# chao1224/GeoSSL

Measured on AMD Instinct MI355X. Metric: molecules/s/GPU SchNet+DDM fwd+bwd (QM9-sized, bs=1024); % HBM roofline, higher is better.
Workload: dtype f32

## Files before the change

geossl_amd/NCSN.py:

```python
import ctypes as C
import os

import numpy as np
import torch
from .switches import env as _env
import torch.nn as nn
import torch.nn.functional as F

from . import _lib
from ._lib import call, ptr, stream
from .layout import get_super_edge_layout


class MultiLayerPerceptron(nn.Module):

    def __init__(self, input_dim, hidden_dims, activation="relu", dropout=0):
        super().__init__()
        self.dims = [input_dim] + hidden_dims
        self.activation = getattr(F, activation) if isinstance(activation, str) else None
        self.dropout = nn.Dropout(dropout) if dropout else None
        self.layers = nn.ModuleList()
        for i in range(len(self.dims) - 1):
            self.layers.append(nn.Linear(self.dims[i], self.dims[i + 1]))
        self.reset_parameters()

    def reset_parameters(self):
        for layer in self.layers:
            nn.init.xavier_uniform_(layer.weight)
            nn.init.constant_(layer.bias, 0.0)

    def forward(self, input):
        from .higher_order import _linear_wide
        _lib.require_cuda(input)
        lead = input.shape[:-1]
        x = input.reshape(-1, input.shape[-1])
        for i, layer in enumerate(self.layers):
            x = _linear_wide(x, layer.weight, layer.bias)
            if i < len(self.layers) - 1:
                if self.activation:
                    x = self.activation(x)
                if self.dropout:
                    x = self.dropout(x)
        return x.reshape(*lead, x.shape[-1])


def _head_params(m):
    i, o = m.input_distance_mlp.layers, m.output_mlp.layers
    return [i[0].weight, i[0].bias, i[1].weight, i[1].bias, o[0].weight, o[0].bias, o[1].weight, o[1].bias,
            o[2].weight, o[2].bias]


_FIELDS = ("in_w1", "in_b1", "in_w2", "in_b2", "o1_w", "o1_b", "o2_w", "o2_b", "o3_w", "o3_b")

_SIDE = {"stream": None, "pending": []}


def set_side_stream(stream):
    _SIDE["stream"] = stream


def join_side_stream():
    if _SIDE["pending"]:
        for ev, _keep in _SIDE["pending"]:
            torch.cuda.current_stream().wait_event(ev)
        _SIDE["pending"].clear()


class _NcsnLoss(torch.autograd.Function):
    @staticmethod
    def forward(ctx, h, distance, noise_level, distance_noise, sel, sigmas, anneal_power, out_scale, *params):
        dev = h.device
        S, Fd = sel.S, h.size(1)
        training = ctx.needs_input_grad[0] or any(ctx.needs_input_grad[8:])
        ps = [p.detach().contiguous() for p in params]
        w = _lib.NcsnWeights()
        for name, p in zip(_FIELDS, ps):
            setattr(w, name, ptr(p))
        w.sigmas = ptr(sigmas)
        ctx.grad_slot = getattr(h, "_geossl_grad_slot", None)
        h = h.detach().contiguous()
        loss_e = torch.empty(S, dtype=torch.float32, device=dev)
        sv = None
        saved = {}
        if training:
            saved = dict(a1=torch.empty(S, Fd, dtype=torch.float32, device=dev),
                         a2=torch.empty(S, Fd // 2, dtype=torch.float32, device=dev),
                         pd=torch.empty(S, dtype=torch.float32, device=dev),
                         emb=torch.empty(S, dtype=torch.float32, device=dev),
                         gscale=torch.empty(S, dtype=torch.float32, device=dev))
            sv = _lib.NcsnSaved(*[ptr(saved[k]) for k in ("a1", "a2", "pd", "emb", "gscale")])
        lib = _lib.load()
        nws = max(int(lib.geossl_ddm_loss_fwd_workspace_floats(Fd)), 256)
        ws = (torch.empty if S > 0 else torch.zeros)(nws, dtype=torch.float32, device=dev)
        st = stream()
        call("geossl_ddm_loss_fwd", ptr(h), ptr(sel.batch), ptr(sel.sei0), ptr(sel.sei1), S,
             ptr(distance.contiguous()), ptr(noise_level.contiguous()), ptr(distance_noise.contiguous()), C.byref(w),
             Fd, float(anneal_power), ptr(loss_e), C.byref(sv) if sv is not None else None, ptr(ws), st)
        loss = torch.empty((), dtype=torch.float32, device=dev)
        call("geossl_loss_reduce_partials", ptr(ws), ptr(sel.stats), float(out_scale), ptr(loss), 0, st)
        if training:
            ctx.sel, ctx.ps, ctx.w, ctx.saved, ctx.h = sel, ps, w, saved, h
            ctx.params = params
            ctx.sigmas = sigmas
            ctx.out_scale = float(out_scale)
        return loss

    @staticmethod
    def backward(ctx, gout):
        sel, ps, w, saved, h = ctx.sel, ctx.ps, ctx.w, ctx.saved, ctx.h
        dev = h.device
        S, Fd, N = sel.S, h.size(1), h.size(0)
        st = stream()
        sv = _lib.NcsnSaved(*[ptr(saved[k]) for k in ("a1", "a2", "pd", "emb", "gscale")])
        dfeat = torch.empty(S, Fd, dtype=torch.float32, device=dev)
        demb = torch.empty(S, dtype=torch.float32, device=dev)
        grow = torch.empty(S, dtype=torch.float32, device=dev)
        gout = gout.contiguous().to(torch.float32)
        direct = _lib.direct_grads_enabled(ctx.params)
        grads = [p.grad for p in ctx.params] if direct else [torch.empty_like(p) for p in ps]
        g = _lib.NcsnGrads(*[ptr(t) for t in grads])
        lib = _lib.load()
        acc = 1 if direct else 0
        split = (_env("GEOSSL_NCSN_SPLIT_BWD") is not None or _env("GEOSSL_ARITH_24BIT") is not None
                 or max(S, N) * Fd * 4 >= 2 ** 32)
        if not split:
            ws1 = torch.empty(int(lib.geossl_ddm_loss_bwd_fused_workspace_floats(S, Fd)), dtype=torch.float32, device=dev)
            call("geossl_ddm_loss_bwd_fused", ptr(h), ptr(sel.sei0), ptr(sel.sei1), S, N, Fd, C.byref(w), C.byref(sv),
                 ptr(sel.stats), ctx.out_scale, ptr(gout), ptr(dfeat), ptr(demb), ptr(grow), C.byref(g), ptr(ws1), acc, st)
            dz1 = None
        else:
            dz1 = torch.empty(S, Fd, dtype=torch.float32, device=dev)
            call("geossl_ddm_loss_bwd_rows", C.byref(w), C.byref(sv), S, Fd, ptr(sel.stats), ctx.out_scale, ptr(gout),
                 ptr(dz1), ptr(dfeat), ptr(demb), ptr(grow), st)
        dh = None
        if ctx.needs_input_grad[0]:
            slot = ctx.grad_slot
            dh = slot.rows(N, Fd, torch.float32, dev) if slot is not None else None
            if dh is None:
                dh = torch.empty(N, Fd, dtype=torch.float32, device=dev)
            call("geossl_incidence_gather", ptr(dfeat), ptr(sel.inc_ptr), ptr(sel.inc_idx), N, Fd, ptr(dh), 0, st)
        if split:
            nfl = lib.geossl_ddm_loss_bwd_workspace_floats(S, Fd)
            side = _SIDE["stream"] if direct else None
            if side is None:
                ws = torch.empty(nfl, dtype=torch.float32, device=dev)
                call("geossl_ddm_loss_bwd_weights", ptr(h), ptr(sel.sei0), ptr(sel.sei1), S, Fd, C.byref(w), C.byref(sv),
                     ptr(dz1), ptr(demb), ptr(grow), C.byref(g), ptr(ws), acc, st)
            else:
                main = torch.cuda.current_stream()
                fork = torch.cuda.Event()
                fork.record(main)
                side.wait_event(fork)
                with torch.cuda.stream(side):
                    ws = torch.empty(nfl, dtype=torch.float32, device=dev)
                    call("geossl_ddm_loss_bwd_weights", ptr(h), ptr(sel.sei0), ptr(sel.sei1), S, Fd, C.byref(w),
                         C.byref(sv), ptr(dz1), ptr(demb), ptr(grow), C.byref(g), ptr(ws), 1, stream())
                    done = torch.cuda.Event()
                    done.record(side)
                _SIDE["pending"].append((done, (h, saved, dz1, demb, grow, ws, w, sv, ps, grads)))
        if direct:
            return (dh, None, None, None, None, None, None, None) + (None,) * len(grads)
        return (dh, None, None, None, None, None, None, None) + tuple(grads)


class _NcsnLossPair(torch.autograd.Function):

    @staticmethod
    def forward(ctx, h1, h2, d1, d2, nl1, dn1, nl2, dn2, sel, sigmas, powers, out_scale, npar, *params):
        dev = h1.device
        S, Fd, N = sel.S, h1.size(1), h1.size(0)
        training = ctx.needs_input_grad[0] or ctx.needs_input_grad[1] or any(ctx.needs_input_grad[13:])
        ps = [p.detach().contiguous() for p in params]
        pss = (ps[:npar], ps[npar:])
        dyn = getattr(sel, "dyn", None)
        ctx.dyn = dyn
        if dyn is not None:
            hs = (h1.detach().contiguous(),) * 2
            ctx.grad_slots = (None, None)
        else:
            hs = (h1.detach().contiguous(), h2.detach().contiguous())
            ctx.grad_slots = (getattr(h1, "_geossl_grad_slot", None), getattr(h2, "_geossl_grad_slot", None))
        heads = (_lib.NcsnHeadFwd * 2)()
        keep, saved, ws = [], [], []
        for k, (h, d, nl, dn) in enumerate(((hs[0], d1, nl1, dn1), (hs[1], d2, nl2, dn2))):
            hd = heads[k]
            d, nl, dn = d.contiguous(), nl.contiguous(), dn.contiguous()
            keep += [d, nl, dn]
            for name, p in zip(_FIELDS, pss[k]):
                setattr(hd.w, name, ptr(p))
            hd.w.sigmas = ptr(sigmas[k])
            hd.h, hd.distance, hd.noise_level, hd.distance_noise = ptr(h), ptr(d), ptr(nl), ptr(dn)
            hd.anneal_power = float(powers[k])
            loss_e = torch.empty(S, dtype=torch.float32, device=dev)
            sv = {}
            if training:
                sv = dict(a1=torch.empty(S, Fd, dtype=torch.float32, device=dev),
                          a2=torch.empty(S, Fd // 2, dtype=torch.float32, device=dev),
                          pd=torch.empty(S, dtype=torch.float32, device=dev),
                          emb=torch.empty(S, dtype=torch.float32, device=dev),
                          gscale=torch.empty(S, dtype=torch.float32, device=dev))
                for name in ("a1", "a2", "pd", "emb", "gscale"):
                    setattr(hd.saved, name, ptr(sv[name]))
            w_ = torch.empty(256, dtype=torch.float32, device=dev)
            hd.loss_e, hd.workspace = ptr(loss_e), ptr(w_)
            keep.append(loss_e)
            saved.append(sv)
            ws.append(w_)
        st = stream()
        call("geossl_ddm_loss_fwd2_dyn", C.byref(heads), ptr(sel.batch), ptr(sel.sei0), ptr(sel.sei1), S, Fd,
             None if dyn is None else dyn.n_super, None if dyn is None else dyn.n_atoms, st)
        loss = torch.empty((), dtype=torch.float32, device=dev)
        call("geossl_loss_reduce_partials2", ptr(ws[0]), ptr(ws[1]), ptr(sel.stats), float(out_scale), float(out_scale),
             ptr(loss), st)
        if training:
            ctx.sel, ctx.pss, ctx.saved, ctx.hs, ctx.sigmas = sel, pss, saved, hs, sigmas
            ctx.params, ctx.npar, ctx.out_scale = params, npar, float(out_scale)
        return loss

    @staticmethod
    def backward(ctx, gout):
        sel, pss, saved, hs = ctx.sel, ctx.pss, ctx.saved, ctx.hs
        dev = hs[0].device
        S, Fd, N = sel.S, hs[0].size(1), hs[0].size(0)
        st = stream()
        gout = gout.contiguous().to(torch.float32)
        direct = _lib.direct_grads_enabled(ctx.params)
        grads = [p.grad for p in ctx.params] if direct else [torch.empty_like(p) for p in pss[0] + pss[1]]
        gs = (grads[:ctx.npar], grads[ctx.npar:])
        lib = _lib.load()
        heads = (_lib.NcsnHeadBwd * 2)()
        keep, dhs = [], []
        nws = int(lib.geossl_ddm_loss_bwd_fused_workspace_floats(S, Fd))
        dyn = ctx.dyn
        dh_all = torch.empty(N, Fd, dtype=torch.float32, device=dev) if dyn is not None else None
        for k in range(2):
            hd = heads[k]
            for name, p in zip(_FIELDS, pss[k]):
                setattr(hd.w, name, ptr(p))
            hd.w.sigmas = ptr(ctx.sigmas[k])
            for name in ("a1", "a2", "pd", "emb", "gscale"):
                setattr(hd.saved, name, ptr(saved[k][name]))
            for name, t_ in zip(_FIELDS, gs[k]):
                setattr(hd.grads, name, ptr(t_))
            dfeat = torch.empty(S, Fd, dtype=torch.float32, device=dev)
            demb = torch.empty(S, dtype=torch.float32, device=dev)
            grow = torch.empty(S, dtype=torch.float32, device=dev)
            ws1 = torch.empty(nws, dtype=torch.float32, device=dev)
            slot = ctx.grad_slots[k]
            dh = dh_all if dyn is not None else (slot.rows(N, Fd, torch.float32, dev) if slot is not None else None)
            if dh is None:
                dh = torch.empty(N, Fd, dtype=torch.float32, device=dev)
            hd.h, hd.out_scale, hd.dfeat, hd.demb, hd.grow, hd.workspace, hd.dh = (
                ptr(hs[k]), ctx.out_scale, ptr(dfeat), ptr(demb), ptr(grow), ptr(ws1), ptr(dh))
            keep += [dfeat, demb, grow, ws1]
            dhs.append(dh)
        call("geossl_ddm_loss_bwd_fused2_dyn", C.byref(heads), ptr(sel.sei0), ptr(sel.sei1), S, sel.N if dyn is not None else N,
             Fd, ptr(sel.stats), ptr(gout), ptr(sel.inc_ptr), ptr(sel.inc_idx), 1 if direct else 0,
             None if dyn is None else dyn.n_super, None if dyn is None else dyn.n_atoms, st)
        head = ((dh_all, None) if dyn is not None else (dhs[0], dhs[1])) + (None,) * 11
        if direct:
            return head + (None,) * len(grads)
        return head + tuple(grads)


def ddm_heads_loss(n1, n2, data, h1, distance_1, h2, distance_2, noise_level_1=None, distance_noise_1=None,
                   noise_level_2=None, distance_noise_2=None, out_scale=0.5):
    ok = (isinstance(n1, NCSN_version_03) and isinstance(n2, NCSN_version_03) and n1.emb_dim == n2.emb_dim
          and n1.emb_dim in (32, 64, 128) and not _env("GEOSSL_NCSN_SPLIT_BWD")
          and not _env("GEOSSL_ARITH_24BIT")
          and not _env("GEOSSL_NCSN_SEPARATE_HEADS")
          and (h2 is None or h1.shape == h2.shape) and not distance_1.requires_grad and not distance_2.requires_grad
          and n1 is not n2 and not ({id(p) for p in _head_params(n1)} & {id(p) for p in _head_params(n2)}))
    if ok:
        S_, N_, Fd = data.super_edge_index.size(1), h1.size(0), h1.size(1)
        ok = S_ > 0 and max(S_, N_) * Fd * 4 < 2 ** 32
    bucket = getattr(data, "_bucket", None)
    if bucket is not None and (not ok or h2 is not None):
        raise _lib.GeosslHipError("a capacity-bucket batch needs the paired NCSN heads on one fused feature tensor")
    if not ok:
        return (n1(data, h1, distance_1, noise_level=noise_level_1, distance_noise=distance_noise_1, out_scale=out_scale) +
                n2(data, h2, distance_2, noise_level=noise_level_2, distance_noise=distance_noise_2, out_scale=out_scale))
    _lib.require_cuda(h1, h2, distance_1, distance_2, n1.sigmas, n2.sigmas)
    n1.device = n2.device = n1.sigmas.device
    num_graphs = data.num_graphs
    sel = bucket.sel if bucket is not None else get_super_edge_layout(data.batch, data.super_edge_index, num_graphs)
    draws = []
    for n_, nl, dn, d in ((n1, noise_level_1, distance_noise_1, distance_1), (n2, noise_level_2, distance_noise_2, distance_2)):
        if nl is None:
            nl = torch.randint(0, n_.sigmas.size(0), (num_graphs,), device=n_.sigmas.device)
        if dn is None:
            dn = torch.randn_like(d)
        draws.append((nl, dn))
    p1, p2 = _head_params(n1), _head_params(n2)
    return _NcsnLossPair.apply(h1, h2, distance_1.view(-1), distance_2.view(-1), draws[0][0], draws[0][1].view(-1),
                               draws[1][0], draws[1][1].view(-1), sel, (n1.sigmas.detach(), n2.sigmas.detach()),
                               (n1.anneal_power, n2.anneal_power), out_scale, len(p1), *p1, *p2)


class NCSN_version_03(torch.nn.Module):
    def __init__(self, emb_dim, sigma_begin, sigma_end, num_noise_level, noise_type, anneal_power):
        super().__init__()
        self.anneal_power = anneal_power
        self.noise_type = noise_type
        self.input_distance_mlp = MultiLayerPerceptron(1, [emb_dim, 1], activation="relu")
        self.output_mlp = MultiLayerPerceptron(1 + emb_dim, [emb_dim, emb_dim // 2, 1])
        sigmas = torch.tensor(np.exp(np.linspace(np.log(sigma_begin), np.log(sigma_end), num_noise_level)),
                              dtype=torch.float32)
        self.sigmas = nn.Parameter(sigmas, requires_grad=False)
        self.emb_dim = emb_dim

    def forward(self, data, node_feature, distance, debug=False, noise_level=None, distance_noise=None,
                out_scale=1.0):
        self.device = self.sigmas.device
        _lib.require_cuda(node_feature, distance, self.sigmas)
        if self.emb_dim not in (32, 64, 128):
            raise NotImplementedError("HIP path supports emb_dim in (32, 64, 128)")
        if distance.requires_grad:
            raise NotImplementedError("gradient w.r.t. distance/positions is not built (SURVEY.md §8(f) N3)")
        num_graphs = data.num_graphs
        sel = get_super_edge_layout(data.batch, data.super_edge_index, num_graphs)
        if noise_level is None:
            noise_level = torch.randint(0, self.sigmas.size(0), (num_graphs,), device=self.device)
        if distance_noise is None:
            distance_noise = torch.randn_like(distance)
        if sel.S == 0:
            raise ValueError("batch has no super edges (scatter_add over an empty index fails in the reference too)")
        loss = _NcsnLoss.apply(node_feature, distance.view(-1), noise_level, distance_noise.view(-1), sel,
                               self.sigmas.detach(), self.anneal_power, out_scale, *_head_params(self))
        if debug:
            print("loss", float(loss))
        return loss
```

geossl_amd/_lib.py:

```python
import ctypes as C
import os

import torch

HERE = os.path.dirname(os.path.abspath(__file__))
LIB_PATH = os.path.join(HERE, "lib", "libgeossl_hip.so")

MAX_L = 12
TN_MAX = 32
EPI_BIAS, EPI_SSP, EPI_RESIDUAL, EPI_MUL_DSSP, CHAIN_SAME_INPUT, CHAIN_NEW_INPUT, CHAIN_ADD_PREV = 1, 2, 4, 8, 16, 32, 64
EPI_SILU, EPI_MUL_DSILU = 128, 256

vp = C.c_void_p
i64 = C.c_int64
i32 = C.c_int
f32 = C.c_float
f64 = C.c_double
u64 = C.c_uint64


class FilterWeights(C.Structure):
    _fields_ = [("w1", vp * MAX_L), ("b1", vp * MAX_L), ("w2", vp * MAX_L), ("b2", vp * MAX_L)]


PREPARE_MAX = 64


class PrepareBatch(C.Structure):
    _fields_ = [("W", vp * PREPARE_MAX), ("image", vp * PREPARE_MAX), ("ldw", i32 * PREPARE_MAX), ("tb", i32 * PREPARE_MAX)]


CHAIN_MAX = 5


class ChainStage(C.Structure):
    _fields_ = [("image", vp), ("bias", vp), ("res", vp), ("tprev", vp), ("out", vp), ("ld", i32), ("flags", i32),
                ("xin", vp), ("ldxin", i32), ("pad_", i32), ("out_act", vp)]


class Chain(C.Structure):
    _fields_ = [("nstage", i32), ("st", ChainStage * CHAIN_MAX)]


LOOP_MAX_OPS = 14


class LoopOp(C.Structure):
    _fields_ = [("kind", i32), ("swap", i32), ("X", vp), ("Wf", vp), ("out", vp), ("chain", Chain)]


class FilterGradIn(C.Structure):
    _fields_ = [("x", vp * MAX_L), ("dagg", vp * MAX_L)]


class FilterGradOut(C.Structure):
    _fields_ = [("dw1", vp * MAX_L), ("db1", vp * MAX_L), ("dw2", vp * MAX_L), ("db2", vp * MAX_L)]


class TnBatch(C.Structure):
    _fields_ = [("A", vp * TN_MAX), ("B", vp * TN_MAX), ("dW", vp * TN_MAX), ("db", vp * TN_MAX)]


class NcsnWeights(C.Structure):
    _fields_ = [(k, vp) for k in ("in_w1", "in_b1", "in_w2", "in_b2", "o1_w", "o1_b", "o2_w", "o2_b", "o3_w", "o3_b",
                                  "sigmas")]


class NcsnGrads(C.Structure):
    _fields_ = [(k, vp) for k in ("in_w1", "in_b1", "in_w2", "in_b2", "o1_w", "o1_b", "o2_w", "o2_b", "o3_w", "o3_b")]


class NcsnSaved(C.Structure):
    _fields_ = [(k, vp) for k in ("a1", "a2", "pd", "emb", "gscale")]


class NcsnHeadFwd(C.Structure):
    _fields_ = [("h", vp), ("distance", vp), ("noise_level", vp), ("distance_noise", vp), ("w", NcsnWeights),
                ("saved", NcsnSaved), ("anneal_power", f32), ("pad_", f32), ("loss_e", vp), ("workspace", vp)]


class NcsnHeadBwd(C.Structure):
    _fields_ = [("h", vp), ("w", NcsnWeights), ("saved", NcsnSaved), ("out_scale", f32), ("pad_", f32), ("dfeat", vp),
                ("demb", vp), ("grow", vp), ("grads", NcsnGrads), ("workspace", vp), ("dh", vp)]


COPY_MAX = 8


class CopyBatch(C.Structure):
    _fields_ = [("dst", vp * COPY_MAX), ("src", vp * COPY_MAX), ("bytes", i64 * COPY_MAX)]


class Gather(C.Structure):
    _fields_ = [(k, vp) for k in ("x_src", "pos_src", "src_off", "mol_ptr", "x_dst", "pos_dst", "batch_dst", "se_ptr", "sei0",
                                  "sei1", "pair_ptr2", "pair_i", "pair_j", "inc_ptr", "inc_idx", "e0_src", "e1_src",
                                  "e_src_off", "e_ptr", "e0_dst", "e1_dst", "zero")] + \
               [("zero_count", i64), ("x_cols", i32), ("option", i32)]


class Mask(C.Structure):
    _fields_ = [(k, vp) for k in ("bond_ptr", "bond_dst", "src_n", "mol_id", "keep_in", "keep_out", "e_src_cnt",
                                  "e_count")] + [("seed", u64), ("max_n", i32), ("pad_", i32)]


P = C.POINTER
PROTOTYPES = {
    "geossl_abi_version": (i32, []),
    "geossl_layout_build": (i32, [vp, i64, i64, vp, vp, vp, vp]),
    "geossl_pair_index_fill": (i32, [vp, vp, i64, vp, vp, vp]),
    "geossl_radius_graph_count": (i32, [vp, vp, i64, i32, f32, i32, vp, vp]),
    "geossl_radius_graph_fill": (i32, [vp, vp, i64, i32, f32, i32, vp, vp, vp, vp, vp]),
    "geossl_pair_geometry": (i32, [vp, vp, vp, i64, i32, f32, i32, f32, vp, vp, vp, vp]),
    "geossl_rbf_fwd": (i32, [vp, i64, vp, i32, f32, vp, vp]),
    "geossl_ssp_fwd": (i32, [vp, i64, vp, vp]),
    "geossl_ssp_bwd": (i32, [vp, vp, i64, vp, vp]),
    "geossl_cfconv_filter_fwd": (i32, [vp, vp, i64, P(FilterWeights), i32, i32, i32, vp, f32, vp, vp, vp]),
    "geossl_cfconv_filter_bwd_workspace_floats": (i64, [i64, i32, i32, i32]),
    "geossl_cfconv_filter_bwd": (i32, [vp, vp, vp, vp, vp, i64, i64, P(FilterWeights), P(FilterGradIn), i32, i32, i32, vp,
                                       f32, vp, P(FilterGradOut), vp, i32, vp]),
    "geossl_cfconv_filter_dpos": (i32, [vp, vp, vp, vp, vp, i64, P(FilterWeights), P(FilterGradIn), i32, i32, i32, vp, f32,
                                        f32, vp, vp, vp, vp]),
    "geossl_pair_position_grad": (i32, [vp, vp, vp, vp, vp, i64, i64, i32, vp, vp]),
    "geossl_cfconv_aggregate": (i32, [vp, vp, vp, vp, vp, vp, i64, i32, i32, i32, vp, vp]),
    "geossl_aggregate_parts": (i32, [i32]),
    "geossl_cfconv_aggregate_work": (i32, [vp, vp, vp, vp, vp, vp, i64, i32, i32, i32, vp, vp]),
    "geossl_pair_product": (i32, [vp, vp, vp, vp, vp, i64, i32, i32, vp, vp]),
    "geossl_linear": (i32, [vp, i32, vp, vp, vp, vp, vp, i32, i64, i32, i32, i32, i32, vp]),
    "geossl_tn_plan": (None, [i64, i32, P(i32), P(i32)]),
    "geossl_tn_workspace_floats": (i64, [i64, i32, i32, i32]),
    "geossl_row_normalize_fwd": (i32, [vp, i64, i32, f32, vp, vp, vp]),
    "geossl_row_normalize_bwd": (i32, [vp, vp, vp, i64, i32, f32, vp, vp]),
    "geossl_atom_tuples": (i32, [vp, vp, i64, i32, vp, vp, vp]),
    "geossl_linear_image_words": (i64, [i32, i32]),
    "geossl_linear_prepare": (i32, [P(PrepareBatch), i32, i32, i32, i32, vp]),
    "geossl_linear_prepared": (i32, [vp, i32, vp, vp, vp, vp, vp, i32, i64, i32, i32, i32, vp]),
    "geossl_chain_image_words": (i64, [i32]),
    "geossl_chain_prepare": (i32, [P(PrepareBatch), i32, i32, i32, vp]),
    "geossl_linear_chain": (i32, [vp, i32, P(Chain), i64, i32, vp]),
    "geossl_linear_wgrad": (i32, [P(TnBatch), i32, i64, i32, i32, i32, i32, i32, vp, i32, vp]),
    "geossl_embedding_fwd": (i32, [vp, i64, vp, i32, i64, i32, vp, vp, vp]),
    "geossl_embedding_bwd_workspace_floats": (i64, [i32, i32]),
    "geossl_embedding_bwd": (i32, [vp, i64, vp, i32, i64, i32, vp, vp, i32, vp]),
    "geossl_segment_reduce_fwd": (i32, [vp, vp, i64, i32, i32, vp, vp]),
    "geossl_segment_reduce_bwd": (i32, [vp, vp, i64, i32, i32, vp, i32, vp]),
    "geossl_axpy": (i32, [vp, vp, f32, i64, vp, vp]),
    "geossl_pair_distance": (i32, [vp, vp, vp, i64, vp, vp]),
    "geossl_super_edge_ptr": (i32, [vp, vp, vp, i64, i64, vp, vp, vp]),
    "geossl_incidence_count": (i32, [vp, vp, vp, vp, i64, i32, vp, vp]),
    "geossl_incidence_fill": (i32, [vp, vp, vp, vp, i64, i32, vp, vp, vp]),
    "geossl_ddm_loss_fwd_workspace_floats": (i64, [i32]),
    "geossl_ddm_loss_fwd": (i32, [vp, vp, vp, vp, i64, vp, vp, vp, P(NcsnWeights), i32, f32, vp, P(NcsnSaved), vp, vp]),
    "geossl_schnet_layer_loop": (i32, [vp, i32, vp, i32, vp, vp, vp, i32, i32, i64, i32, i32, vp]),
    "geossl_schnet_layer_loop_ragged": (i32, [vp, i32, vp, vp, vp, i64, i32, i64, i32, vp]),
    "geossl_copy2": (i32, [vp, vp, i64, vp, vp, i64, vp]),
    "geossl_ddm_noise": (i32, [vp, f32, f32, i64, i64, i64, i32, i32, vp, vp, vp, vp, vp, vp]),
    "geossl_ddm_noise_seeded": (i32, [u64, f32, f32, i64, i64, i64, i32, i32, vp, vp, vp, vp, vp, vp]),
    "geossl_ddm_views": (i32, [vp, vp, vp, vp, i64, i64, vp, vp, vp, vp, i64, vp, vp]),
    "geossl_loss_reduce_partials": (i32, [vp, vp, f32, vp, i32, vp]),
    "geossl_ddm_loss_fwd2": (i32, [vp, vp, vp, vp, i64, i32, vp]),
    "geossl_loss_reduce_partials2": (i32, [vp, vp, vp, f32, f32, vp, vp]),
    "geossl_ddm_loss_bwd_fused2": (i32, [vp, vp, vp, i64, i64, i32, vp, vp, vp, vp, i32, vp]),
    "geossl_loss_reduce_workspace_floats": (i64, [i64]),
    "geossl_loss_reduce": (i32, [vp, i64, vp, f32, vp, vp, i32, vp]),
    "geossl_ddm_loss_bwd_rows": (i32, [P(NcsnWeights), P(NcsnSaved), i64, i32, vp, f32, vp, vp, vp, vp, vp, vp]),
    "geossl_ddm_loss_bwd_workspace_floats": (i64, [i64, i32]),
    "geossl_ddm_loss_bwd_weights": (i32, [vp, vp, vp, i64, i32, P(NcsnWeights), P(NcsnSaved), vp, vp, vp, P(NcsnGrads),
                                          vp, i32, vp]),
    "geossl_ddm_loss_bwd_fused_workspace_floats": (i64, [i64, i32]),
    "geossl_ddm_loss_bwd_fused": (i32, [vp, vp, vp, i64, i64, i32, P(NcsnWeights), P(NcsnSaved), vp, f32, vp, vp, vp, vp,
                                        P(NcsnGrads), vp, i32, vp]),
    "geossl_incidence_gather": (i32, [vp, vp, vp, i64, i32, vp, i32, vp]),
    "geossl_painn_edge_geom": (i32, [vp, vp, vp, i64, f32, vp, vp, i32, vp, vp, vp, vp]),
    "geossl_silu_fwd": (i32, [vp, i64, vp, vp]),
    "geossl_silu_bwd": (i32, [vp, vp, i64, vp, vp]),
    "geossl_painn_interaction_fwd": (i32, [vp, vp, vp, vp, vp, vp, vp, vp, vp, vp, vp, i64, i32, i32, vp, vp, vp]),
    "geossl_painn_interaction_bwd_workspace_floats": (i64, [i64, i32, i32]),
    "geossl_painn_interaction_fwd_mol": (i32, [vp, vp, vp, vp, vp, vp, vp, vp, vp, vp, vp, vp, i64, i32, i64, i32, i32, vp,
                                               vp, vp]),
    "geossl_painn_interaction_fwd_mma": (i32, [vp, vp, vp, vp, vp, vp, vp, vp, vp, vp, vp, vp, vp, i64, i32, i64, i32, i32,
                                               vp, vp, vp]),
    "geossl_painn_interaction_bwd_mol_workspace_floats": (i64, [i64, i64, i32, i32]),
    "geossl_painn_interaction_bwd_mol": (i32, [vp, vp, vp, vp, vp, vp, vp, vp, vp, vp, vp, vp, vp, i64, i32, i64, i32, i32,
                                               vp, vp, vp, vp, vp, i32, vp]),
    "geossl_painn_interaction_bwd": (i32, [vp, vp, vp, vp, vp, vp, vp, vp, vp, vp, vp, vp, i64, i32, i32, vp, vp, vp, vp,
                                           vp, i32, vp]),
    "geossl_painn_mix_pre_fwd": (i32, [vp, vp, i64, i32, f32, vp, vp, vp]),
    "geossl_painn_mix_post_fwd": (i32, [vp, vp, vp, vp, vp, i64, i32, vp, vp, vp]),
    "geossl_painn_mix_post_bwd": (i32, [vp, vp, vp, vp, vp, i64, i32, vp, vp, vp]),
    "geossl_painn_mix_pre_bwd": (i32, [vp, vp, vp, vp, i64, i32, vp, vp, vp]),
    "geossl_add": (i32, [vp, vp, i64, vp, vp]),
    "geossl_painn_edge_grads": (i32, [vp] * 11 + [i64, i32, i32, vp, vp, vp, i32, vp]),
    "geossl_painn_edge_geom_bwd": (i32, [vp, vp, vp, i64, f32, vp, vp, i32, vp, vp, vp, vp, vp]),
    "geossl_painn_position_grad": (i32, [vp, vp, vp, vp, vp, i64, vp, vp]),
    "geossl_adam_step": (i32, [vp, vp, vp, vp, i64, f64, f64, f64, f64, f64, i64, f32, vp]),
    "geossl_copy_n": (i32, [P(CopyBatch), i32, vp]),
    "geossl_ddm_views_dyn": (i32, [vp, vp, vp, vp, i64, i64, vp, vp, vp, vp, i64, vp, vp, vp, vp]),
    "geossl_embedding_fwd_dyn": (i32, [vp, i64, vp, i32, i64, i32, vp, vp, vp, vp]),
    "geossl_embedding_bwd_dyn": (i32, [vp, i64, vp, i32, i64, i32, vp, vp, i32, vp, vp]),
    "geossl_cfconv_filter_fwd_dyn": (i32, [vp, vp, i64, P(FilterWeights), i32, i32, i32, vp, f32, vp, vp, vp, vp]),
    "geossl_cfconv_filter_bwd_dyn": (i32, [vp, vp, vp, vp, vp, i64, i64, P(FilterWeights), P(FilterGradIn), i32, i32, i32,
                                           vp, f32, vp, P(FilterGradOut), vp, i32, vp, vp, vp]),
    "geossl_cfconv_aggregate_work_dyn": (i32, [vp, vp, vp, vp, vp, vp, i64, i32, i32, i32, vp, vp, vp]),
    "geossl_cfconv_aggregate_targets_dyn": (i32, [vp, vp, vp, vp, vp, vp, i64, i32, i32, i32, vp, vp, vp]),
    "geossl_linear_chain_dyn": (i32, [vp, i32, P(Chain), i64, i32, vp, vp]),
    "geossl_linear_wgrad_dyn": (i32, [P(TnBatch), i32, i64, i32, i32, i32, i32, i32, vp, i32, vp, vp]),
    "geossl_ddm_loss_fwd2_dyn": (i32, [vp, vp, vp, vp, i64, i32, vp, vp, vp]),
    "geossl_ddm_loss_bwd_fused2_dyn": (i32, [vp, vp, vp, i64, i64, i32, vp, vp, vp, vp, i32, vp, vp, vp]),
    "geossl_painn_group_capacity": (i64, [i64, i64]),
    "geossl_painn_edge_layout": (i32, [vp, vp, i64, vp, i64, i64, i64] + [vp] * 12),
    "geossl_painn_edge_layout_dyn": (i32, [vp, vp, i64, vp, vp, i64, i64, i64] + [vp] * 12),
    "geossl_painn_edge_geom_dyn": (i32, [vp, vp, vp, i64, f32, vp, vp, i32, vp, vp, vp, vp, vp]),
    "geossl_painn_interaction_fwd_mma_dyn": (i32, [vp, vp, vp, vp, vp, vp, vp, vp, vp, vp, vp, vp, vp, i64, i32, i64, i32,
                                                   i32, vp, vp, vp, vp]),
    "geossl_tape_unary": (i32, [i32, vp, i64, f32, f32, vp, vp]),
    "geossl_tape_binary": (i32, [i32, vp, i32, vp, i32, i64, i32, f32, vp, vp]),
    "geossl_tape_colsum_workspace_floats": (i64, [i64, i32]),
    "geossl_tape_reduce": (i32, [i32, vp, i64, i32, vp, vp, vp]),
    "geossl_tape_gather_rows": (i32, [vp, vp, i32, i64, i32, vp, vp]),
    "geossl_tape_scatter_rows": (i32, [vp, vp, i32, vp, i64, i32, vp, vp]),
    "geossl_tape_copy2d": (i32, [vp, i64, vp, i64, i64, i32, vp]),
    "geossl_tape_fill": (i32, [vp, i64, f32, vp]),
    "geossl_painn_stage_cap": (i32, [i32, i32, i32]),
    "geossl_painn_interaction_fwd_atoms": (i32, [vp] * 12 + [i64, vp, i32, i32, vp, vp, vp]),
    "geossl_painn_interaction_bwd_atoms": (i32, [vp] * 13 + [i64, vp, i32, i32, vp, vp, vp, vp, vp, i32, vp]),
    "geossl_painn_interaction_bwd_mol_skip": (i32, [vp, vp, vp, vp, vp, vp, vp, vp, vp, vp, vp, vp, vp, i64, i32, i64, i32,
                                                    i32, vp, vp, vp, vp, vp, i32, vp]),
    "geossl_painn_mix_pre_fwd_dyn": (i32, [vp, vp, i64, i32, f32, vp, vp, vp, vp]),
    "geossl_painn_mix_post_fwd_dyn": (i32, [vp, vp, vp, vp, vp, i64, i32, vp, vp, vp, vp]),
    "geossl_painn_mix_post_bwd_dyn": (i32, [vp, vp, vp, vp, vp, i64, i32, vp, vp, vp, vp]),
    "geossl_painn_mix_pre_bwd_dyn": (i32, [vp, vp, vp, vp, i64, i32, vp, vp, vp, vp]),
    "geossl_gather_molecules": (i32, [P(Gather), i64, vp]),
    "geossl_gather_masked_molecules": (i32, [P(Gather), P(Mask), i64, vp]),
    "geossl_masked_edge_offsets": (i32, [vp, i64, i64, i32, vp, vp, vp, vp]),
    "geossl_infonce_fwd": (i32, [vp, vp, i64, i32, f32, vp, vp, vp, vp, vp]),
    "geossl_infonce_bwd": (i32, [vp, vp, vp, vp, i64, i32, f32, vp, vp, vp, vp]),
    "geossl_ebm_nce_fwd": (i32, [vp, vp, i64, i32, i32, vp, vp, vp, vp, vp, vp]),
    "geossl_ebm_nce_bwd": (i32, [vp, vp, vp, i64, i32, i32, vp, vp, vp, vp]),
    "geossl_distance_head_width_ok": (i32, [i32]),
    "geossl_distance_head_fwd_workspace_floats": (i64, [i64]),
    "geossl_distance_head_bwd_workspace_floats": (i64, [i64, i32]),
    "geossl_distance_head_fwd": (i32, [vp, i64, i32, vp, vp, vp, vp, vp, i64, vp, vp, vp, vp, vp, vp]),
    "geossl_distance_head_fwd_dyn": (i32, [vp, i64, i32, vp, vp, vp, vp, vp, i64, vp, vp, vp, vp, vp, vp, vp, vp]),
    "geossl_distance_head_bwd": (i32, [vp, i64, i32, vp, vp, i64, vp, vp, vp, vp, vp, vp, vp, vp, i32, vp]),
    "geossl_distance_head_bwd_dyn": (i32, [vp, i64, i32, vp, vp, i64, vp, vp, vp, vp, vp, vp, vp, vp, i32, vp, vp, vp]),
    "geossl_charge_mask_count": (i64, [i64, f64]),
    "geossl_charge_mask": (i32, [vp, i32, i64, f64, i32, vp, vp, vp, vp, vp, vp]),
    "geossl_charge_mask_dyn": (i32, [vp, i32, i64, f64, i32, vp, vp, vp, vp, vp, vp, vp]),
    "geossl_charge_head_width_ok": (i32, [i32, i32]),
    "geossl_charge_head_fwd_workspace_floats": (i64, [i64]),
    "geossl_charge_head_bwd_workspace_floats": (i64, [i64, i32, i32]),
    "geossl_charge_head_fwd": (i32, [vp, i64, i32, vp, vp, i32, vp, vp, i64, vp, vp, vp, vp, vp, vp]),
    "geossl_charge_head_fwd_dyn": (i32, [vp, i64, i32, vp, vp, i32, vp, vp, i64, vp, vp, vp, vp, vp, vp, vp]),
    "geossl_charge_head_bwd": (i32, [vp, i64, i32, vp, i32, vp, vp, i64, vp, vp, vp, vp, vp, vp, vp, i32, vp]),
    "geossl_charge_head_bwd_dyn": (i32, [vp, i64, i32, vp, i32, vp, vp, i64, vp, vp, vp, vp, vp, vp, vp, i32, vp, vp]),
    "geossl_infograph_width_ok": (i32, [i32]),
    "geossl_infograph_fwd_workspace_floats": (i64, [i64]),
    "geossl_infograph_fwd": (i32, [vp, i64, i32, vp, vp, i64, i32, vp, vp, vp, vp, vp, vp, vp, vp]),
    "geossl_infograph_fwd_dyn": (i32, [vp, i64, i32, vp, vp, i64, i32, vp, vp, vp, vp, vp, vp, vp, vp, vp]),
    "geossl_infograph_bwd": (i32, [vp, i64, i32, vp, vp, i64, i32, vp, vp, vp, vp, vp, vp, vp, vp]),
    "geossl_infograph_bwd_dyn": (i32, [vp, i64, i32, vp, vp, i64, i32, vp, vp, vp, vp, vp, vp, vp, vp, vp]),
    "geossl_property_width_ok": (i32, [i32]),
    "geossl_property_workspace_floats": (i64, [i64]),
    "geossl_property_fwd": (i32, [vp, i64, i32, vp, i64, i32, i32, vp, vp, vp, vp, vp, i64, vp, i32, vp, vp, vp, vp, vp,
                                  vp]),
    "geossl_property_fwd_dyn": (i32, [vp, i64, i32, vp, i64, i32, i32, vp, vp, vp, vp, vp, i64, vp, i32, vp, vp, vp, vp,
                                      vp, vp, vp]),
    "geossl_property_predict": (i32, [vp, i64, i32, vp, i64, i32, i32, vp, vp, vp, vp, vp, vp, vp]),
    "geossl_property_predict_dyn": (i32, [vp, i64, i32, vp, i64, i32, i32, vp, vp, vp, vp, vp, vp, vp, vp]),
    "geossl_property_bwd": (i32, [i64, i32, vp, i64, i32, i32, vp, vp, vp, vp, vp, vp, i64, vp, i32, vp, vp, vp, vp, vp,
                                  vp, i32, vp]),
    "geossl_property_bwd_dyn": (i32, [i64, i32, vp, i64, i32, i32, vp, vp, vp, vp, vp, vp, i64, vp, i32, vp, vp, vp, vp,
                                      vp, vp, i32, vp, vp]),
    "geossl_property_targets": (i32, [vp, i64, i32, i32, vp, vp, i64, vp, vp]),
    "geossl_pair_head_width_ok": (i32, [i32]),
    "geossl_pair_head_workspace_floats": (i64, [i64]),
    "geossl_pair_head_fwd": (i32, [vp, i64, i32, vp, i64, i32, vp, vp, vp, vp, vp, vp, vp, vp]),
    "geossl_pair_head_predict": (i32, [vp, i64, i32, vp, i64, i32, vp, vp, vp, vp]),
    "geossl_pair_head_bwd": (i32, [i64, i32, vp, i64, i32, vp, vp, vp, vp, vp, vp, vp, vp, vp, i32, vp]),
    "geossl_torsion_head_width_ok": (i32, [i32]),
    "geossl_torsion_head_fwd_workspace_floats": (i64, [i64]),
    "geossl_torsion_head_bwd_workspace_floats": (i64, [i64, i32]),
    "geossl_torsion_head_fwd": (i32, [vp, i64, i32, vp, vp, vp, vp, vp, vp, i64, vp, vp, vp, vp, vp, vp]),
    "geossl_torsion_head_fwd_dyn": (i32, [vp, i64, i32, vp, vp, vp, vp, vp, vp, i64, vp, vp, vp, vp, vp, vp, vp, vp]),
    "geossl_torsion_head_bwd": (i32, [vp, i64, i32, vp, vp, vp, vp, i64, vp, vp, i64, vp, vp, vp, vp, vp, i32, vp]),
    "geossl_torsion_head_bwd_dyn": (i32, [vp, i64, i32, vp, vp, vp, vp, i64, vp, vp, i64, vp, vp, vp, vp, vp, i32, vp, vp,
                                          vp]),
    "geossl_triple_angles": (i32, [vp, i64, vp, vp, vp, i64, vp, vp]),
    "geossl_gather_triples": (i32, [vp, i64, vp, vp, vp, vp, i64, vp, vp, vp, vp, vp]),
    "geossl_sparse_pairs_build": (i32, [vp, vp, i64, i64, i32, f32, i32, f32, i64] + [vp] * 13),
    "geossl_cfconv_aggregate_sparse": (i32, [vp, vp, vp, vp, vp, i64, i32, i32, vp, vp]),
    "geossl_pair_position_grad_sparse": (i32, [vp, vp, vp, vp, vp, vp, i64, i64, i32, vp, vp]),
    "geossl_pair_geometry_live": (i32, [vp, vp, vp, i64, i32, f32, i32, f32, vp, vp, vp, vp, vp]),
    "geossl_gather_live_rows": (i32, [vp, vp, vp, i64, i32, i32, vp, vp]),
    "geossl_live_pairs_build": (i32, [vp] * 8 + [i64, i64, f32] + [vp] * 9),
    "geossl_cfconv_filter_fwd_rows": (i32, [vp, vp, i64, P(FilterWeights), i32, i32, i32, vp, f32, vp, vp, vp, vp, vp]),
}

_lib = None


class GeosslHipError(RuntimeError):
    pass


def load():
    global _lib
    if _lib is not None:
        return _lib
    path = os.environ.get("GEOSSL_HIP_LIB", LIB_PATH)
    if not os.path.exists(path):
        raise GeosslHipError(
            "libgeossl_hip.so is not built (%s). Run `python -m geossl_amd.build` (needs hipcc); "
            "there is no CPU fallback." % path)
    lib = C.CDLL(path)
    for name, (res, args) in PROTOTYPES.items():
        fn = getattr(lib, name)
        fn.restype = res
        fn.argtypes = args
    if lib.geossl_abi_version() != 1:
        raise GeosslHipError("ABI version mismatch")
    _lib = lib
    return lib


def check(rc, what):
    if rc != 0:
        raise GeosslHipError("%s failed with hipError %d" % (what, rc))


def ptr(t):
    if t is None:
        return None
    return t.data_ptr()


def stream():
    return torch._C._cuda_getCurrentRawStream(torch._C._cuda_getDevice())


def require_cuda(*tensors):
    for t in tensors:
        if t is not None and not t.is_cuda:
            raise GeosslHipError(
                "geossl_amd runs on MI355X only: got a %s tensor. The HIP path has no CPU fallback." % t.device.type)



_DIRECT = {"depth": 0}


class direct_grads:
    def __enter__(self):
        _DIRECT["depth"] += 1
        return self

    def __exit__(self, *exc):
        _DIRECT["depth"] -= 1
        return False


def direct_grads_enabled(params):
    return _DIRECT["depth"] > 0 and all(
        p.grad is not None and p.grad.is_contiguous() and p.grad.dtype == torch.float32 and p.grad.is_cuda
        for p in params)


class StatusWord:

    def __init__(self, device, message):
        self.word = torch.zeros(1, dtype=torch.int32, device=device)
        self.host = torch.zeros(1, dtype=torch.int32).pin_memory()
        self.event = None
        self.message = message

    def __deepcopy__(self, memo):
        return None

    def __reduce__(self):
        return (type(None), ())

    def poll(self):
        if self.event is None or torch.cuda.is_current_stream_capturing():
            return
        if self.event.query():
            self.event = None
            if int(self.host[0]):
                raise IndexError(self.message)

    def arm(self, every=1):
        self.calls = getattr(self, "calls", 0) + 1
        if every > 1 and self.calls % every != 1:
            return
        if self.event is None and not torch.cuda.is_current_stream_capturing():
            self.host.copy_(self.word, non_blocking=True)
            self.event = torch.cuda.Event()
            self.event.record()

    def check(self):
        if int(self.word.item()):
            raise IndexError(self.message)


def module_status(module, device, message):
    st = module.__dict__.get("_geossl_status")
    if st is None or st.word.device != device:
        st = StatusWord(device, message)
        module.__dict__["_geossl_status"] = st
    return st


TIMERS = None
CALLS = None


def call(name, *args):
    global CALLS
    lib = load()
    if CALLS is not None:
        CALLS += 1
    timers = TIMERS
    key = name[:-4] if name.endswith("_dyn") else name
    if key == "geossl_cfconv_filter_fwd_rows":
        key = "geossl_cfconv_filter_fwd"
    if timers is not None and key in timers:
        e0, e1 = torch.cuda.Event(enable_timing=True), torch.cuda.Event(enable_timing=True)
        e0.record()
        rc = getattr(lib, name)(*args)
        e1.record()
        timers[key].append((e0, e1))
    else:
        rc = getattr(lib, name)(*args)
    check(rc, name)


def fill_ptrs(arr, tensors):
    for i, t in enumerate(tensors):
        arr[i] = ptr(t)
```

geossl_amd/build.py:

```python
import os
import subprocess
import sys

HERE = os.path.dirname(os.path.abspath(__file__))
REPO = os.path.dirname(HERE)
CSRC = os.path.join(HERE, "csrc")
LIB_DIR = os.path.join(HERE, "lib")
LIB_PATH = os.path.join(LIB_DIR, "libgeossl_hip.so")


def _sources():
    return sorted(f for f in os.listdir(CSRC) if f.endswith(".hip"))


SOURCE_FLAGS = {"painn_mma.hip": ["-fno-slp-vectorize"], "distance_head.hip": ["-fno-slp-vectorize"],
                "charge_head.hip": ["-fno-slp-vectorize"], "infograph_head.hip": ["-fno-slp-vectorize"],
                "property_head.hip": ["-fno-slp-vectorize"], "torsion_head.hip": ["-fno-slp-vectorize"],
                "pair_head.hip": ["-fno-slp-vectorize"]}


def _headers():
    hs = [os.path.join(CSRC, f) for f in os.listdir(CSRC) if f.endswith(".h")]
    inc = os.path.join(REPO, "include")
    return hs + [os.path.join(inc, f) for f in os.listdir(inc) if f.endswith(".h")]


def source_hash():
    import hashlib
    h = hashlib.sha256()
    h.update(repr(sorted(SOURCE_FLAGS.items())).encode())
    for path in sorted([os.path.join(CSRC, s_) for s_ in _sources()] + _headers()):
        h.update(os.path.basename(path).encode() + b"\0")
        with open(path, "rb") as fh:
            h.update(fh.read())
    return h.hexdigest()[:16]


def _newest(paths):
    return max(os.path.getmtime(p) for p in paths)


def needs_build():
    if not os.path.exists(LIB_PATH):
        return True
    deps = [os.path.join(CSRC, s) for s in _sources()] + _headers() + [os.path.abspath(__file__)]
    return _newest(deps) > os.path.getmtime(LIB_PATH)


def build(force=False, verbose=True):
    if not force and not needs_build():
        return LIB_PATH
    os.makedirs(LIB_DIR, exist_ok=True)
    hipcc = os.environ.get("HIPCC", "/opt/rocm/bin/hipcc")
    objs = []
    procs = []
    for s in _sources():
        obj = os.path.join(LIB_DIR, s.replace(".hip", ".o"))
        cmd = [hipcc, "--offload-arch=gfx950", "-O3", "-std=c++17", "-fPIC", "-I", os.path.join(REPO, "include"),
               "-I", CSRC, "-Wno-pass-failed"] + SOURCE_FLAGS.get(s, []) + ["-c", os.path.join(CSRC, s), "-o", obj]
        if verbose:
            print(" ".join(cmd), flush=True)
        procs.append((cmd, subprocess.Popen(cmd)))
        objs.append(obj)
    for cmd, p in procs:
        if p.wait() != 0:
            raise RuntimeError("hipcc failed: " + " ".join(cmd))
    cmd = [hipcc, "--offload-arch=gfx950", "-shared", "-fPIC", "-o", LIB_PATH] + objs
    if verbose:
        print(" ".join(cmd), flush=True)
    subprocess.check_call(cmd)
    return LIB_PATH


if __name__ == "__main__":
    build(force="--force" in sys.argv)
    print(LIB_PATH)
```

geossl_amd/csrc/ncsn_rows.hip:

```cpp
#include "common.h"
#include "geossl_hip.h"
#include "split.h"

using namespace geossl;

namespace {

struct RowIn {
  int64_t u, v;
  float sigma, d, eps;
};

template <int NMB>
__device__ __forceinline__ void ncsn_fwd_body(const float* __restrict__ h, const int64_t* __restrict__ batch,
                                              const int64_t* __restrict__ sei0, const int64_t* __restrict__ sei1,
                                              int S, const float* __restrict__ distance,
                                              const int64_t* __restrict__ noise_level,
                                              const float* __restrict__ dist_noise, const GeosslNcsnWeights& w,
                                              float anneal_power, float* __restrict__ loss_e,
                                              const GeosslNcsnSaved& sv, float* __restrict__ loss_part) {
  constexpr int F = 32 * NMB, H = F / 2, HMB = (H + 31) / 32, HP = 32 * HMB, KS = F / 16;
  extern __shared__ __attribute__((aligned(16))) uint8_t smem_raw[];
  u32x4* W1f = reinterpret_cast<u32x4*>(smem_raw);
  u32x4* W2f = W1f + NMB * KS * 3 * 64;
  float* b1s = reinterpret_cast<float*>(W2f + HMB * KS * 3 * 64);
  float* wls = b1s + F;
  float* b2s = wls + F;
  float* w3s = b2s + HP;
  float* iw1 = w3s + HP;
  float* ib1 = iw1 + F;
  float* iw2 = ib1 + F;
  float* lred = iw2 + F;
  const int tid = threadIdx.x, lane = tid & 63, wave = tid >> 6, j = lane & 31, kh = lane >> 5;
  const int nrb = (S + 31) / 32;
  float lsum = 0.0f;
  auto load_row = [&](int rb) {
    RowIn r;
    const int rowc = min(32 * rb + j, S - 1);
    r.u = sei0[rowc];
    r.v = sei1[rowc];
    r.sigma = w.sigmas[noise_level[batch[r.u]]];
    r.d = distance[rowc];
    r.eps = dist_noise[rowc];
    return r;
  };
  int rb = blockIdx.x + gridDim.x * wave;
  RowIn cur;
  if (rb < nrb) cur = load_row(rb);
#ifdef NCSN_STAGE_UNROLL
#pragma unroll
#endif
  for (int i = tid; i < NMB * KS * 64; i += 512) {
    const int ln = i & 63, ks = (i >> 6) % KS, mb = i / (64 * KS);
    const float* row = w.o1_w + (size_t)(32 * mb + (ln & 31)) * (F + 1) + 16 * ks + 8 * (ln >> 5);
    float v[8];
#pragma unroll
    for (int e = 0; e < 8; ++e) v[e] = row[e];
    const Frag3 f = split8(v);
    u32x4* dst = W1f + ((size_t)(mb * KS + ks) * 3) * 64 + ln;
    dst[0] = f.h;
    dst[64] = f.m;
    dst[128] = f.l;
  }
#ifdef NCSN_STAGE_UNROLL
#pragma unroll
#endif
  for (int i = tid; i < HMB * KS * 64; i += 512) {
    const int ln = i & 63, ks = (i >> 6) % KS, mb = i / (64 * KS);
    const int m = 32 * mb + (ln & 31);
    const float* row = w.o2_w + (size_t)min(m, H - 1) * F + 16 * ks + 4 * (ln >> 5);
    const f32x4 lo = *reinterpret_cast<const f32x4*>(row), hi = *reinterpret_cast<const f32x4*>(row + 8);
    float v[8] = {lo.x, lo.y, lo.z, lo.w, hi.x, hi.y, hi.z, hi.w};
    if (m >= H) {
#pragma unroll
      for (int e = 0; e < 8; ++e) v[e] = 0.0f;
    }
    const Frag3 f = split8(v);
    u32x4* dst = W2f + ((size_t)(mb * KS + ks) * 3) * 64 + ln;
    dst[0] = f.h;
    dst[64] = f.m;
    dst[128] = f.l;
  }
  for (int i = tid; i < F; i += 512) {
    b1s[i] = w.o1_b[i];
    wls[i] = w.o1_w[(size_t)i * (F + 1) + F];
    iw1[i] = w.in_w1[i];
    ib1[i] = w.in_b1[i];
    iw2[i] = w.in_w2[i];
  }
  for (int i = tid; i < HP; i += 512) {
    b2s[i] = i < H ? w.o2_b[i] : 0.0f;
    w3s[i] = i < H ? w.o3_w[i] : 0.0f;
  }
  __syncthreads();
  const float ib2 = w.in_b2[0], b3 = w.o3_b[0];
  for (; rb < nrb; rb += gridDim.x * 8) {
    const int row = 32 * rb + j;
    const bool valid = row < S;
    const RowIn in = cur;
    f32x4 gq[2][4];
    auto gather = [&](int ks, f32x4 (&g)[4]) {
      const float* hu = h + (size_t)in.u * F + 16 * ks + 8 * kh;
      const float* hv = h + (size_t)in.v * F + 16 * ks + 8 * kh;
      g[0] = *reinterpret_cast<const f32x4*>(hu);
      g[1] = *reinterpret_cast<const f32x4*>(hu + 4);
      g[2] = *reinterpret_cast<const f32x4*>(hv);
      g[3] = *reinterpret_cast<const f32x4*>(hv + 4);
    };
    gather(0, gq[0]);
    if (rb + gridDim.x * 8 < nrb) cur = load_row(rb + gridDim.x * 8);
    const float pd = add_rn(in.d, mul_rn(in.eps, in.sigma));
    float e = 0.0f;
#pragma unroll 4
    for (int k = kh * (F / 2); k < (kh + 1) * (F / 2); k += 4) {
      const f32x4 a = *reinterpret_cast<const f32x4*>(iw1 + k), b = *reinterpret_cast<const f32x4*>(ib1 + k);
      const f32x4 c = *reinterpret_cast<const f32x4*>(iw2 + k);
      e = fmaf(c.x, fmaxf(fmaf(a.x, pd, b.x), 0.0f), e);
      e = fmaf(c.y, fmaxf(fmaf(a.y, pd, b.y), 0.0f), e);
      e = fmaf(c.z, fmaxf(fmaf(a.z, pd, b.z), 0.0f), e);
      e = fmaf(c.w, fmaxf(fmaf(a.w, pd, b.w), 0.0f), e);
    }
    e += __shfl_xor(e, 32, 64);
    const float emb = e + ib2;
    f32x16 acc1[NMB];
#pragma unroll
    for (int mb = 0; mb < NMB; ++mb)
#pragma unroll
      for (int q = 0; q < 4; ++q) {
        const f32x4 b = *reinterpret_cast<const f32x4*>(b1s + 32 * mb + 8 * q + 4 * kh);
        const f32x4 wl = *reinterpret_cast<const f32x4*>(wls + 32 * mb + 8 * q + 4 * kh);
        acc1[mb][4 * q] = fmaf(emb, wl.x, b.x);
        acc1[mb][4 * q + 1] = fmaf(emb, wl.y, b.y);
        acc1[mb][4 * q + 2] = fmaf(emb, wl.z, b.z);
        acc1[mb][4 * q + 3] = fmaf(emb, wl.w, b.w);
      }
#pragma unroll
    for (int ks = 0; ks < KS; ++ks) {
      if (ks + 1 < KS) gather(ks + 1, gq[(ks + 1) & 1]);
      const f32x4(&g)[4] = gq[ks & 1];
      const float v[8] = {g[0].x + g[2].x, g[0].y + g[2].y, g[0].z + g[2].z, g[0].w + g[2].w,
                          g[1].x + g[3].x, g[1].y + g[3].y, g[1].z + g[3].z, g[1].w + g[3].w};
      const Frag3 bf = split8(v);
      Frag3 af[NMB];
#pragma unroll
      for (int mb = 0; mb < NMB; ++mb) {
        const u32x4* src = W1f + ((size_t)(mb * KS + ks) * 3) * 64 + lane;
        af[mb].h = src[0];
        af[mb].m = src[64];
        af[mb].l = src[128];
      }
#pragma unroll
      for (int mb = 0; mb < NMB; ++mb) acc1[mb] = mfma_bf16(af[mb].l, bf.h, acc1[mb]);
#pragma unroll
      for (int mb = 0; mb < NMB; ++mb) acc1[mb] = mfma_bf16(af[mb].h, bf.l, acc1[mb]);
#pragma unroll
      for (int mb = 0; mb < NMB; ++mb) acc1[mb] = mfma_bf16(af[mb].m, bf.m, acc1[mb]);
#pragma unroll
      for (int mb = 0; mb < NMB; ++mb) acc1[mb] = mfma_bf16(af[mb].m, bf.h, acc1[mb]);
#pragma unroll
      for (int mb = 0; mb < NMB; ++mb) acc1[mb] = mfma_bf16(af[mb].h, bf.m, acc1[mb]);
#pragma unroll
      for (int mb = 0; mb < NMB; ++mb) acc1[mb] = mfma_bf16(af[mb].h, bf.h, acc1[mb]);
      __builtin_amdgcn_sched_barrier(0);
    }
    Frag3 tb[KS];
    {
      float* arow = sv.a1 != nullptr ? sv.a1 + (size_t)row * F + 4 * kh : nullptr;
#pragma unroll
      for (int mb = 0; mb < NMB; ++mb)
#pragma unroll
        for (int half = 0; half < 2; ++half) {
          float v[8];
#pragma unroll
          for (int e2 = 0; e2 < 8; ++e2) v[e2] = fmaxf(acc1[mb][8 * half + e2], 0.0f);
          if (arow != nullptr && valid) {
            *reinterpret_cast<f32x4*>(arow + 32 * mb + 16 * half) = f32x4{v[0], v[1], v[2], v[3]};
            *reinterpret_cast<f32x4*>(arow + 32 * mb + 16 * half + 8) = f32x4{v[4], v[5], v[6], v[7]};
          }
          tb[2 * mb + half] = split8(v);
          __builtin_amdgcn_sched_barrier(0);
        }
    }
    float sc = 0.0f;
#pragma unroll
    for (int mb = 0; mb < HMB; ++mb) {
      f32x16 acc2;
#pragma unroll
      for (int q = 0; q < 4; ++q) {
        const f32x4 b = *reinterpret_cast<const f32x4*>(b2s + 32 * mb + 8 * q + 4 * kh);
        acc2[4 * q] = b.x;
        acc2[4 * q + 1] = b.y;
        acc2[4 * q + 2] = b.z;
        acc2[4 * q + 3] = b.w;
      }
      Frag3 af, an;
      {
        const u32x4* src = W2f + ((size_t)(mb * KS) * 3) * 64 + lane;
        af.h = src[0]; af.m = src[64]; af.l = src[128];
      }
#pragma unroll
      for (int ks = 0; ks < KS; ++ks) {
        if (ks + 1 < KS) {
          const u32x4* src = W2f + ((size_t)(mb * KS + ks + 1) * 3) * 64 + lane;
          an.h = src[0]; an.m = src[64]; an.l = src[128];
        }
        __builtin_amdgcn_sched_barrier(0);
        mma6(acc2, af, tb[ks]);
        __builtin_amdgcn_sched_barrier(0);
        if (ks + 1 < KS) af = an;
      }
      float* a2row = sv.a2 != nullptr ? sv.a2 + (size_t)row * H + 32 * mb + 4 * kh : nullptr;
#pragma unroll
      for (int q = 0; q < 4; ++q) {
        const f32x4 w3 = *reinterpret_cast<const f32x4*>(w3s + 32 * mb + 8 * q + 4 * kh);
        const f32x4 a = f32x4{fmaxf(acc2[4 * q], 0.0f), fmaxf(acc2[4 * q + 1], 0.0f), fmaxf(acc2[4 * q + 2], 0.0f),
                              fmaxf(acc2[4 * q + 3], 0.0f)};
        sc = fmaf(a.x, w3.x, sc);
        sc = fmaf(a.y, w3.y, sc);
        sc = fmaf(a.z, w3.z, sc);
        sc = fmaf(a.w, w3.w, sc);
        if (a2row != nullptr && valid && 32 * mb + 8 * q + 4 * kh < H) *reinterpret_cast<f32x4*>(a2row + 8 * q) = a;
      }
    }
    sc += __shfl_xor(sc, 32, 64);
    const float out = sc + b3;
    const float inv_sigma = 1.0f / in.sigma;
    const float score = out * inv_sigma;
    const float target = (-1.0f / (in.sigma * in.sigma)) * (pd - in.d);
    const float diff = score - target;
    const float pw = powf(in.sigma, anneal_power);
    if (valid && kh == 0) {
      const float le = (0.5f * (diff * diff)) * pw;
      loss_e[row] = le;
      lsum += le;
      if (sv.pd != nullptr) {
        sv.pd[row] = pd;
        sv.emb[row] = emb;
        sv.gscale[row] = diff * pw * inv_sigma;
      }
    }
  }
  if (loss_part != nullptr) {
    lsum = wave_sum(lsum);
    if (lane == 0) lred[wave] = lsum;
    __syncthreads();
    if (tid == 0) {
      float t = 0.0f;
      for (int i = 0; i < 8; ++i) t += lred[i];
      loss_part[blockIdx.x] = t;
    }
    if (blockIdx.x == 0)
      for (int i = (int)gridDim.x + tid; i < GEOSSL_LOSS_PARTIALS; i += 512) loss_part[i] = 0.0f;
  }
}

template <int NMB>
__global__ __launch_bounds__(512) void k_ncsn_fwd(const float* __restrict__ h, const int64_t* __restrict__ batch,
                                                  const int64_t* __restrict__ sei0, const int64_t* __restrict__ sei1,
                                                  int S, const float* __restrict__ distance,
                                                  const int64_t* __restrict__ noise_level,
                                                  const float* __restrict__ dist_noise, GeosslNcsnWeights w,
                                                  float anneal_power, float* __restrict__ loss_e,
                                                  GeosslNcsnSaved sv, float* __restrict__ loss_part) {
  ncsn_fwd_body<NMB>(h, batch, sei0, sei1, S, distance, noise_level, dist_noise, w, anneal_power, loss_e, sv, loss_part);
}
struct NcsnFwdHead {
  const float* h;
  const float* distance;
  const int64_t* noise_level;
  const float* dist_noise;
  GeosslNcsnWeights w;
  GeosslNcsnSaved sv;
  float anneal_power;
  float* loss_e;
  float* loss_part;
};
struct NcsnFwdPair { NcsnFwdHead a[2]; };
template <int NMB>
__global__ __launch_bounds__(512) void k_ncsn_fwd2(NcsnFwdPair pr, const int64_t* __restrict__ batch,
                                                   const int64_t* __restrict__ sei0, const int64_t* __restrict__ sei1,
                                                   int S, const int32_t* __restrict__ dyn_S,
                                                   const int32_t* __restrict__ dyn_view) {
  const NcsnFwdHead& a = pr.a[blockIdx.y];
  const float* h = a.h;
  if (dyn_view != nullptr && blockIdx.y == 1) h += (size_t)(*dyn_view) * (32 * NMB);
  ncsn_fwd_body<NMB>(h, batch, sei0, sei1, dyn_count(S, dyn_S), a.distance, a.noise_level, a.dist_noise, a.w,
                     a.anneal_power, a.loss_e, a.sv, a.loss_part);
}

template <int NMB>
__global__ __launch_bounds__(512) void k_ncsn_bwd_rows(GeosslNcsnWeights w, GeosslNcsnSaved sv, int S,
                                                       const int64_t* __restrict__ divisor, float out_scale,
                                                       const float* __restrict__ gout, float* __restrict__ dz1,
                                                       float* __restrict__ dfeat, float* __restrict__ demb,
                                                       float* __restrict__ grow) {
  constexpr int F = 32 * NMB, H = F / 2, HP = 32 * ((H + 31) / 32), KS = F / 16, KH = H / 16;
  extern __shared__ __attribute__((aligned(16))) uint8_t smem_raw[];
  u32x4* W2t = reinterpret_cast<u32x4*>(smem_raw);
  u32x4* W1t = W2t + NMB * KH * 3 * 64;
  float* wls = reinterpret_cast<float*>(W1t + NMB * KS * 3 * 64);
  float* w3s = wls + F;
  const int tid = threadIdx.x, lane = tid & 63, wave = tid >> 6, j = lane & 31, kh = lane >> 5;
  for (int i = tid; i < NMB * KH * 64; i += 512) {
    const int ln = i & 63, ks = (i >> 6) % KH, mb = i / (64 * KH);
    const float* col = w.o2_w + (size_t)(16 * ks + 8 * (ln >> 5)) * F + 32 * mb + (ln & 31);
    float v[8];
#pragma unroll
    for (int e = 0; e < 8; ++e) v[e] = col[(size_t)e * F];
    const Frag3 f = split8(v);
    u32x4* dst = W2t + ((size_t)(mb * KH + ks) * 3) * 64 + ln;
    dst[0] = f.h;
    dst[64] = f.m;
    dst[128] = f.l;
  }
  for (int i = tid; i < NMB * KS * 64; i += 512) {
    const int ln = i & 63, ks = (i >> 6) % KS, mb = i / (64 * KS);
    const float* col = w.o1_w + 32 * mb + (ln & 31);
    float v[8];
#pragma unroll
    for (int e = 0; e < 8; ++e) v[e] = col[(size_t)(16 * ks + kperm(e, ln >> 5)) * (F + 1)];
    const Frag3 f = split8(v);
    u32x4* dst = W1t + ((size_t)(mb * KS + ks) * 3) * 64 + ln;
    dst[0] = f.h;
    dst[64] = f.m;
    dst[128] = f.l;
  }
  for (int i = tid; i < F; i += 512) wls[i] = w.o1_w[(size_t)i * (F + 1) + F];
  for (int i = tid; i < HP; i += 512) w3s[i] = i < H ? w.o3_w[i] : 0.0f;
  __syncthreads();
  const float scale = out_scale * (gout != nullptr ? gout[0] : 1.0f) / (float)divisor[0];
  const int nrb = (S + 31) / 32;
  for (int rb = blockIdx.x + gridDim.x * wave; rb < nrb; rb += gridDim.x * 8) {
    const int row = 32 * rb + j;
    const bool valid = row < S;
    const size_t rowc = (size_t)min(row, S - 1);
    const float gr = valid ? sv.gscale[rowc] * scale : 0.0f;
    if (valid && kh == 0) grow[row] = gr;
    Frag3 zb[KH];
    {
      const float* a2row = sv.a2 + rowc * H + 8 * kh;
      f32x4 a2v[KH][2];
#pragma unroll
      for (int ks = 0; ks < KH; ++ks) {
        a2v[ks][0] = *reinterpret_cast<const f32x4*>(a2row + 16 * ks);
        a2v[ks][1] = *reinterpret_cast<const f32x4*>(a2row + 16 * ks + 4);
      }
#pragma unroll
      for (int ks = 0; ks < KH; ++ks) {
        const f32x4 w0 = *reinterpret_cast<const f32x4*>(w3s + 16 * ks + 8 * kh);
        const f32x4 w1 = *reinterpret_cast<const f32x4*>(w3s + 16 * ks + 8 * kh + 4);
        const f32x4 a0 = a2v[ks][0], a1 = a2v[ks][1];
        const float v[8] = {a0.x > 0.0f ? gr * w0.x : 0.0f, a0.y > 0.0f ? gr * w0.y : 0.0f,
                            a0.z > 0.0f ? gr * w0.z : 0.0f, a0.w > 0.0f ? gr * w0.w : 0.0f,
                            a1.x > 0.0f ? gr * w1.x : 0.0f, a1.y > 0.0f ? gr * w1.y : 0.0f,
                            a1.z > 0.0f ? gr * w1.z : 0.0f, a1.w > 0.0f ? gr * w1.w : 0.0f};
        zb[ks] = split8(v);
      }
    }
    f32x4 a1v[NMB][4];
    {
      const float* a1row = sv.a1 + rowc * F + 4 * kh;
#pragma unroll
      for (int mb = 0; mb < NMB; ++mb)
#pragma unroll
        for (int q = 0; q < 4; ++q) a1v[mb][q] = *reinterpret_cast<const f32x4*>(a1row + 32 * mb + 8 * q);
    }
    f32x16 acc[NMB];
#pragma unroll
    for (int mb = 0; mb < NMB; ++mb)
#pragma unroll
      for (int r = 0; r < 16; ++r) acc[mb][r] = 0.0f;
#pragma unroll
    for (int ks = 0; ks < KH; ++ks) {
      Frag3 af[NMB];
#pragma unroll
      for (int mb = 0; mb < NMB; ++mb) {
        const u32x4* src = W2t + ((size_t)(mb * KH + ks) * 3) * 64 + lane;
        af[mb].h = src[0];
        af[mb].m = src[64];
        af[mb].l = src[128];
      }
#pragma unroll
      for (int mb = 0; mb < NMB; ++mb) acc[mb] = mfma_bf16(af[mb].l, zb[ks].h, acc[mb]);
#pragma unroll
      for (int mb = 0; mb < NMB; ++mb) acc[mb] = mfma_bf16(af[mb].h, zb[ks].l, acc[mb]);
#pragma unroll
      for (int mb = 0; mb < NMB; ++mb) acc[mb] = mfma_bf16(af[mb].m, zb[ks].m, acc[mb]);
#pragma unroll
      for (int mb = 0; mb < NMB; ++mb) acc[mb] = mfma_bf16(af[mb].m, zb[ks].h, acc[mb]);
#pragma unroll
      for (int mb = 0; mb < NMB; ++mb) acc[mb] = mfma_bf16(af[mb].h, zb[ks].m, acc[mb]);
#pragma unroll
      for (int mb = 0; mb < NMB; ++mb) acc[mb] = mfma_bf16(af[mb].h, zb[ks].h, acc[mb]);
      __builtin_amdgcn_sched_barrier(0);
    }
    Frag3 tb[KS];
    float de = 0.0f;
    {
      float* zrow = dz1 + (size_t)row * F + 4 * kh;
#pragma unroll
      for (int mb = 0; mb < NMB; ++mb)
#pragma unroll
        for (int half = 0; half < 2; ++half) {
          float v[8];
#pragma unroll
          for (int q2 = 0; q2 < 2; ++q2) {
            const f32x4 a = a1v[mb][2 * half + q2];
            const f32x4 wl = *reinterpret_cast<const f32x4*>(wls + 32 * mb + 16 * half + 8 * q2 + 4 * kh);
            v[4 * q2] = a.x > 0.0f ? acc[mb][8 * half + 4 * q2] : 0.0f;
            v[4 * q2 + 1] = a.y > 0.0f ? acc[mb][8 * half + 4 * q2 + 1] : 0.0f;
            v[4 * q2 + 2] = a.z > 0.0f ? acc[mb][8 * half + 4 * q2 + 2] : 0.0f;
            v[4 * q2 + 3] = a.w > 0.0f ? acc[mb][8 * half + 4 * q2 + 3] : 0.0f;
            de = fmaf(v[4 * q2], wl.x, de);
            de = fmaf(v[4 * q2 + 1], wl.y, de);
            de = fmaf(v[4 * q2 + 2], wl.z, de);
            de = fmaf(v[4 * q2 + 3], wl.w, de);
          }
          if (valid) {
            *reinterpret_cast<f32x4*>(zrow + 32 * mb + 16 * half) = f32x4{v[0], v[1], v[2], v[3]};
            *reinterpret_cast<f32x4*>(zrow + 32 * mb + 16 * half + 8) = f32x4{v[4], v[5], v[6], v[7]};
          }
          tb[2 * mb + half] = split8(v);
          __builtin_amdgcn_sched_barrier(0);
        }
    }
    de += __shfl_xor(de, 32, 64);
    if (valid && kh == 0) demb[row] = de;
    float* frow = dfeat + (size_t)row * F + 4 * kh;
    constexpr int MP = NMB >= 2 ? 2 : 1;
#pragma unroll
    for (int mb0 = 0; mb0 < NMB; mb0 += MP) {
      f32x16 acc2[MP];
#pragma unroll
      for (int u = 0; u < MP; ++u)
#pragma unroll
        for (int r = 0; r < 16; ++r) acc2[u][r] = 0.0f;
      Frag3 af[MP], an[MP];
#pragma unroll
      for (int u = 0; u < MP; ++u) {
        const u32x4* src = W1t + ((size_t)((mb0 + u) * KS) * 3) * 64 + lane;
        af[u].h = src[0]; af[u].m = src[64]; af[u].l = src[128];
      }
#pragma unroll
      for (int ks = 0; ks < KS; ++ks) {
        if (ks + 1 < KS) {
#pragma unroll
          for (int u = 0; u < MP; ++u) {
            const u32x4* src = W1t + ((size_t)((mb0 + u) * KS + ks + 1) * 3) * 64 + lane;
            an[u].h = src[0]; an[u].m = src[64]; an[u].l = src[128];
          }
        }
        __builtin_amdgcn_sched_barrier(0);
#pragma unroll
        for (int u = 0; u < MP; ++u) acc2[u] = mfma_bf16(af[u].l, tb[ks].h, acc2[u]);
#pragma unroll
        for (int u = 0; u < MP; ++u) acc2[u] = mfma_bf16(af[u].h, tb[ks].l, acc2[u]);
#pragma unroll
        for (int u = 0; u < MP; ++u) acc2[u] = mfma_bf16(af[u].m, tb[ks].m, acc2[u]);
#pragma unroll
        for (int u = 0; u < MP; ++u) acc2[u] = mfma_bf16(af[u].m, tb[ks].h, acc2[u]);
#pragma unroll
        for (int u = 0; u < MP; ++u) acc2[u] = mfma_bf16(af[u].h, tb[ks].m, acc2[u]);
#pragma unroll
        for (int u = 0; u < MP; ++u) acc2[u] = mfma_bf16(af[u].h, tb[ks].h, acc2[u]);
        __builtin_amdgcn_sched_barrier(0);
        if (ks + 1 < KS) {
#pragma unroll
          for (int u = 0; u < MP; ++u) af[u] = an[u];
        }
      }
      if (valid) {
#pragma unroll
        for (int u = 0; u < MP; ++u)
#pragma unroll
          for (int q = 0; q < 4; ++q)
            *reinterpret_cast<f32x4*>(frow + 32 * (mb0 + u) + 8 * q) =
                f32x4{acc2[u][4 * q], acc2[u][4 * q + 1], acc2[u][4 * q + 2], acc2[u][4 * q + 3]};
      }
    }
  }
}

inline int row_blocks_grid(int64_t S) {
  const int nrb = (int)((S + 31) / 32);
  int nx = (nrb + 7) / 8;
  return nx < 256 ? nx : 256;
}

}

extern "C" int64_t geossl_ddm_loss_fwd_workspace_floats(int F) { return GEOSSL_LOSS_PARTIALS; }

extern "C" int geossl_ddm_loss_fwd(const float* h, const int64_t* batch, const int64_t* sei0, const int64_t* sei1,
                                   int64_t S, const float* distance, const int64_t* noise_level,
                                   const float* distance_noise, const GeosslNcsnWeights* w, int F, float anneal_power,
                                   float* loss_e, const GeosslNcsnSaved* saved, float* workspace, hipStream_t stream) {
  if (S <= 0) return 0;
  if (F != 32 && F != 64 && F != 128) return (int)hipErrorInvalidValue;
  GeosslNcsnSaved sv = {nullptr, nullptr, nullptr, nullptr, nullptr};
  if (saved != nullptr) sv = *saved;
  const int NMB = F / 32, H = F / 2, HMB = (H + 31) / 32, KS = F / 16;
  const size_t lds = (size_t)(NMB + HMB) * KS * 3 * 1024 + (size_t)(5 * F + 2 * 32 * HMB + 8) * sizeof(float);
  dim3 grid(row_blocks_grid(S));
#define LAUNCH(NMBV)                                                                                              \
  do {                                                                                                            \
    allow_big_lds(&k_ncsn_fwd<NMBV>);                                                                             \
    hipLaunchKernelGGL((k_ncsn_fwd<NMBV>), grid, dim3(512), lds, stream, h, batch, sei0, sei1, (int)S, distance,  \
                       noise_level, distance_noise, *w, anneal_power, loss_e, sv, workspace);                     \
  } while (0)
  if (F == 128) LAUNCH(4); else if (F == 64) LAUNCH(2); else LAUNCH(1);
#undef LAUNCH
  GEOSSL_CHECK_LAUNCH();
  return 0;
}

extern "C" int geossl_ddm_loss_fwd2(const GeosslNcsnHeadFwd* heads, const int64_t* batch, const int64_t* sei0,
                                    const int64_t* sei1, int64_t S, int F, hipStream_t stream) {
  return geossl_ddm_loss_fwd2_dyn(heads, batch, sei0, sei1, S, F, nullptr, nullptr, stream);
}

extern "C" int geossl_ddm_loss_fwd2_dyn(const GeosslNcsnHeadFwd* heads, const int64_t* batch, const int64_t* sei0,
                                        const int64_t* sei1, int64_t S, int F, const int32_t* dyn_S,
                                        const int32_t* dyn_view, hipStream_t stream) {
  if (S <= 0) return 0;
  if (heads == nullptr || (F != 32 && F != 64 && F != 128)) return (int)hipErrorInvalidValue;
  NcsnFwdPair pr;
  NcsnFwdHead* a = pr.a;
  for (int k = 0; k < 2; ++k) {
    const GeosslNcsnHeadFwd& hd = heads[k];
    if (hd.h == nullptr || hd.loss_e == nullptr) return (int)hipErrorInvalidValue;
    a[k].h = hd.h; a[k].distance = hd.distance; a[k].noise_level = hd.noise_level; a[k].dist_noise = hd.distance_noise;
    a[k].w = hd.w; a[k].sv = hd.saved; a[k].anneal_power = hd.anneal_power; a[k].loss_e = hd.loss_e;
    a[k].loss_part = hd.workspace;
  }
  const int NMB = F / 32, H = F / 2, HMB = (H + 31) / 32, KS = F / 16;
  const size_t lds = (size_t)(NMB + HMB) * KS * 3 * 1024 + (size_t)(5 * F + 2 * 32 * HMB + 8) * sizeof(float);
  dim3 grid((row_blocks_grid(S) + 1) / 2, 2);
#define LAUNCH(NMBV)                                                                                              \
  do {                                                                                                            \
    allow_big_lds(&k_ncsn_fwd2<NMBV>);                                                                            \
    hipLaunchKernelGGL((k_ncsn_fwd2<NMBV>), grid, dim3(512), lds, stream, pr, batch, sei0, sei1, (int)S,           \
                       dyn_S, dyn_view);                                                                          \
  } while (0)
  if (F == 128) LAUNCH(4); else if (F == 64) LAUNCH(2); else LAUNCH(1);
#undef LAUNCH
  GEOSSL_CHECK_LAUNCH();
  return 0;
}

extern "C" int geossl_ddm_loss_bwd_rows(const GeosslNcsnWeights* w, const GeosslNcsnSaved* saved, int64_t S, int F,
                                        const int64_t* stats_divisor, float out_scale, const float* gout, float* dz1,
                                        float* dfeat, float* demb, float* grow, hipStream_t stream) {
  if (S <= 0) return 0;
  if (F != 32 && F != 64 && F != 128) return (int)hipErrorInvalidValue;
  const int NMB = F / 32, H = F / 2, KS = F / 16, KH = H / 16;
  const size_t lds = (size_t)NMB * (KS + KH) * 3 * 1024 + (size_t)(F + 32 * ((H + 31) / 32)) * sizeof(float);
  dim3 grid(row_blocks_grid(S));
#define LAUNCH(NMBV)                                                                                              \
  do {                                                                                                            \
    allow_big_lds(&k_ncsn_bwd_rows<NMBV>);                                                                        \
    hipLaunchKernelGGL((k_ncsn_bwd_rows<NMBV>), grid, dim3(512), lds, stream, *w, *saved, (int)S, stats_divisor,  \
                       out_scale, gout, dz1, dfeat, demb, grow);                                                  \
  } while (0)
  if (F == 128) LAUNCH(4); else if (F == 64) LAUNCH(2); else LAUNCH(1);
#undef LAUNCH
  GEOSSL_CHECK_LAUNCH();
  return 0;
}
```

include/geossl_hip.h:

```cpp
#ifndef GEOSSL_HIP_H
#define GEOSSL_HIP_H
#include <stdint.h>
#ifdef __HIPCC__
#include <hip/hip_runtime.h>
#else
typedef struct ihipStream_t* hipStream_t;
#endif

#ifdef __cplusplus
extern "C" {
#endif

#define GEOSSL_ABI_VERSION 1
#define GEOSSL_MAX_L 12
#define GEOSSL_TN_MAX 32
#define GEOSSL_LOSS_PARTIALS 256

#define GEOSSL_EPI_BIAS 1
#define GEOSSL_EPI_SSP 2
#define GEOSSL_EPI_RESIDUAL 4
#define GEOSSL_EPI_MUL_DSSP 8
#define GEOSSL_CHAIN_NEW_INPUT 32
#define GEOSSL_CHAIN_ADD_PREV 64
#define GEOSSL_EPI_SILU 128
#define GEOSSL_EPI_MUL_DSILU 256
#define GEOSSL_CHAIN_SAME_INPUT 16

int geossl_abi_version(void);

int geossl_layout_build(const int64_t* batch, int64_t N, int64_t B, int32_t* mol_ptr, int32_t* pair_ptr,
                        int64_t* stats, hipStream_t stream);
int geossl_atom_tuples(const int32_t* mol_ptr, const int64_t* tuple_ptr, int64_t B, int option, int64_t* out0,
                       int64_t* out1, hipStream_t stream);
int geossl_pair_index_fill(const int32_t* mol_ptr, const int32_t* pair_ptr, int64_t B, int32_t* pair_i,
                           int32_t* pair_j, hipStream_t stream);

int geossl_radius_graph_count(const float* pos, const int32_t* mol_ptr, int64_t B, int max_n, float r2, int cap,
                              int32_t* deg, hipStream_t stream);
int geossl_radius_graph_fill(const float* pos, const int32_t* mol_ptr, int64_t B, int max_n, float r2, int cap,
                             const int64_t* edge_ptr, int64_t* edge_src, int64_t* edge_dst, float* edge_weight,
                             hipStream_t stream);
int geossl_pair_geometry(const float* pos, const int32_t* mol_ptr, const int32_t* pair_ptr, int64_t B, int max_n,
                         float r2, int cap, float cutoff, float* pair_d, float* pair_c, uint8_t* pair_flag,
                         hipStream_t stream);

int geossl_rbf_fwd(const float* d, int64_t E, const float* offset, int G, float coeff, float* out,
                   hipStream_t stream);

int geossl_ssp_fwd(const float* x, int64_t n, float* y, hipStream_t stream);
int geossl_ssp_bwd(const float* y, const float* dy, int64_t n, float* dx, hipStream_t stream);

typedef struct {
  const float* w1[GEOSSL_MAX_L];
  const float* b1[GEOSSL_MAX_L];
  const float* w2[GEOSSL_MAX_L];
  const float* b2[GEOSSL_MAX_L];
} GeosslFilterWeights;
int geossl_cfconv_filter_fwd(const float* pair_d, const float* pair_c, int64_t P, const GeosslFilterWeights* w, int L,
                             int F, int G, const float* offset, float coeff, float* T, float* Wf, hipStream_t stream);

typedef struct {
  const float* x[GEOSSL_MAX_L];
  const float* dagg[GEOSSL_MAX_L];
} GeosslFilterGradIn;
typedef struct {
  float* dw1[GEOSSL_MAX_L];
  float* db1[GEOSSL_MAX_L];
  float* dw2[GEOSSL_MAX_L];
  float* db2[GEOSSL_MAX_L];
} GeosslFilterGradOut;
int64_t geossl_cfconv_filter_bwd_workspace_floats(int64_t P, int L, int F, int G);
int geossl_cfconv_filter_bwd(const float* pair_d, const float* pair_c, const uint8_t* pair_flag, const int32_t* pair_i,
                             const int32_t* pair_j, int64_t P, int64_t N, const GeosslFilterWeights* w,
                             const GeosslFilterGradIn* g, int L, int F, int G, const float* offset, float coeff,
                             const float* T, const GeosslFilterGradOut* out, float* workspace, int accumulate,
                             hipStream_t stream);

int geossl_cfconv_filter_dpos(const float* pair_d, const float* pair_c, const uint8_t* pair_flag, const int32_t* pair_i,
                              const int32_t* pair_j, int64_t P, const GeosslFilterWeights* w,
                              const GeosslFilterGradIn* g, int L, int F, int G, const float* offset, float coeff,
                              float cutoff, const float* T, const float* Wf, float* dd, hipStream_t stream);
int geossl_pair_position_grad(const float* pos, const float* pair_d, const float* dd, const int32_t* mol_ptr,
                              const int32_t* pair_ptr, int64_t B, int64_t P, int L, float* dpos, hipStream_t stream);

int geossl_cfconv_aggregate(const float* x, const float* Wf, const uint8_t* pair_flag, const int32_t* mol_ptr,
                            const int32_t* pair_ptr, const int32_t* order, int64_t B, int max_n, int F, int swap,
                            float* out, hipStream_t stream);
int geossl_aggregate_parts(int n);
int geossl_cfconv_aggregate_targets_dyn(const float* x, const float* Wf, const uint8_t* pair_flag, const int32_t* mol_ptr,
                                        const int32_t* pair_ptr, const int32_t* work, int64_t nwork, int max_n, int F,
                                        int swap, float* out, const int32_t* dyn_nwork, hipStream_t stream);
int geossl_cfconv_aggregate_work(const float* x, const float* Wf, const uint8_t* pair_flag, const int32_t* mol_ptr,
                                 const int32_t* pair_ptr, const int32_t* work, int64_t nwork, int max_n, int F,
                                 int swap, float* out, hipStream_t stream);

int geossl_pair_product(const float* a, const float* b, const int32_t* pair_i, const int32_t* pair_j,
                        const uint8_t* pair_flag, int64_t P, int F, int swap, float* out, hipStream_t stream);

int geossl_linear(const float* X, int ldx, const float* W, const float* bias, const float* res, const float* tprev,
                  float* Y, int ldy, int64_t R, int K, int NO, int transB, int flags, hipStream_t stream);

#define GEOSSL_PREPARE_MAX 64
typedef struct {
  const float* W[GEOSSL_PREPARE_MAX];
  uint32_t* image[GEOSSL_PREPARE_MAX];
  int ldw[GEOSSL_PREPARE_MAX];
  int tb[GEOSSL_PREPARE_MAX];
} GeosslPrepareBatch;
int64_t geossl_linear_image_words(int K, int NO);
int geossl_linear_prepare(const GeosslPrepareBatch* batch, int nprob, int K, int NO, int transB, hipStream_t stream);
int geossl_linear_prepared(const float* X, int ldx, const uint32_t* image, const float* bias, const float* res,
                           const float* tprev, float* Y, int ldy, int64_t R, int K, int NO, int flags,
                           hipStream_t stream);

#define GEOSSL_CHAIN_MAX 5
typedef struct {
  const uint32_t* image;
  const float* bias;
  const float* res;
  const float* tprev;
  float* out;
  int ld;
  int flags;
  const float* xin;
  int ldxin;
  int pad_;
  float* out_act;
} GeosslChainStage;
typedef struct {
  int nstage;
  GeosslChainStage st[GEOSSL_CHAIN_MAX];
} GeosslChain;
int64_t geossl_chain_image_words(int F);
int geossl_chain_prepare(const GeosslPrepareBatch* batch, int nprob, int F, int transB, hipStream_t stream);
int geossl_linear_chain(const float* X, int ldx, const GeosslChain* chain, int64_t R, int F, hipStream_t stream);

#define GEOSSL_LOOP_MAX_OPS 14
typedef struct {
  int kind;
  int swap;
  const float* X;
  const float* Wf;
  float* out;
  GeosslChain chain;
} GeosslLoopOp;
int geossl_schnet_layer_loop(const GeosslLoopOp* ops, int nops, const int32_t* plan, int nblocks, const int32_t* mol_ptr,
                             const int32_t* pair_ptr, const uint8_t* pair_flag, int max_n, int uniform, int64_t N, int F,
                             int stagger, hipStream_t stream);
int geossl_schnet_layer_loop_ragged(const GeosslLoopOp* ops, int nops, const int32_t* mol_ptr, const int32_t* pair_ptr,
                                    const uint8_t* pair_flag, int64_t B, int mols_per_block, int64_t N, int F,
                                    hipStream_t stream);

typedef struct {
  const float* A[GEOSSL_TN_MAX];
  const float* B[GEOSSL_TN_MAX];
  float* dW[GEOSSL_TN_MAX];
  float* db[GEOSSL_TN_MAX];
} GeosslTnBatch;
typedef struct {
  float* out[GEOSSL_TN_MAX];
} GeosslReduceBatch;
void geossl_tn_plan(int64_t R, int nprob, int* chunk, int* nblk);
int64_t geossl_tn_workspace_floats(int64_t R, int M, int N, int nprob);
int geossl_linear_wgrad(const GeosslTnBatch* batch, int nprob, int64_t R, int M, int N, int lda, int ldb, int ldw,
                        float* workspace, int accumulate, hipStream_t stream);

int geossl_embedding_fwd(const int64_t* z, int64_t z_stride, const float* table, int num_classes, int64_t N, int F,
                         float* out, int32_t* status, hipStream_t stream);
int64_t geossl_embedding_bwd_workspace_floats(int num_classes, int F);
int geossl_embedding_bwd(const int64_t* z, int64_t z_stride, const float* dh, int num_classes, int64_t N, int F,
                         float* dtable, float* workspace, int accumulate, hipStream_t stream);

int geossl_segment_reduce_fwd(const float* h, const int32_t* mol_ptr, int64_t B, int F, int mean, float* out,
                              hipStream_t stream);
int geossl_row_normalize_fwd(const float* h, int64_t N, int F, float eps, float* y, float* norm, hipStream_t stream);
int geossl_row_normalize_bwd(const float* g, const float* y, const float* norm, int64_t N, int F, float eps,
                             float* dh, hipStream_t stream);
int geossl_segment_reduce_bwd(const float* dout, const int32_t* mol_ptr, int64_t B, int F, int mean, float* dh,
                              int accumulate, hipStream_t stream);

int geossl_axpy(const float* a, const float* b, float alpha, int64_t n, float* out, hipStream_t stream);
int geossl_pair_distance(const float* pos, const int64_t* sei0, const int64_t* sei1, int64_t S, float* out,
                         hipStream_t stream);
int geossl_copy2(void* dst0, const void* src0, int64_t bytes0, void* dst1, const void* src1, int64_t bytes1,
                 hipStream_t stream);
int geossl_ddm_noise(const int64_t* seed, float mu, float sigma, int64_t n_pos, int64_t S, int64_t B, int K1, int K2,
                     float* pos_noise, int64_t* noise_level_1, float* distance_noise_1, int64_t* noise_level_2,
                     float* distance_noise_2, hipStream_t stream);
int geossl_ddm_noise_seeded(uint64_t seed, float mu, float sigma, int64_t n_pos, int64_t S, int64_t B, int K1, int K2,
                            float* pos_noise, int64_t* noise_level_1, float* distance_noise_1, int64_t* noise_level_2,
                            float* distance_noise_2, hipStream_t stream);
int geossl_ddm_views(const float* pos, const float* noise, const int64_t* sei0, const int64_t* sei1, int64_t N, int64_t S,
                     float* pos2, float* d01, float* d02, const int64_t* z, int64_t z_stride, int64_t* z2,
                     hipStream_t stream);
int geossl_super_edge_ptr(const int64_t* batch, const int64_t* sei0, const int64_t* sei1, int64_t S, int64_t B,
                          int32_t* se_ptr, int64_t* stats, hipStream_t stream);
int geossl_incidence_count(const int64_t* batch, const int64_t* sei0, const int64_t* sei1, const int32_t* se_ptr,
                           int64_t N, int sides, int32_t* inc_cnt, hipStream_t stream);
int geossl_incidence_fill(const int64_t* batch, const int64_t* sei0, const int64_t* sei1, const int32_t* se_ptr,
                          int64_t N, int sides, const int64_t* inc_ptr, int32_t* inc_idx, hipStream_t stream);

typedef struct {
  const float* in_w1;
  const float* in_b1;
  const float* in_w2;
  const float* in_b2;
  const float* o1_w;
  const float* o1_b;
  const float* o2_w;
  const float* o2_b;
  const float* o3_w;
  const float* o3_b;
  const float* sigmas;
} GeosslNcsnWeights;
typedef struct {
  float* in_w1; float* in_b1; float* in_w2; float* in_b2;
  float* o1_w; float* o1_b; float* o2_w; float* o2_b; float* o3_w; float* o3_b;
} GeosslNcsnGrads;
typedef struct {
  float* a1; float* a2; float* pd; float* emb; float* gscale;
} GeosslNcsnSaved;
int64_t geossl_ddm_loss_fwd_workspace_floats(int F);
int geossl_ddm_loss_fwd(const float* h, const int64_t* batch, const int64_t* sei0, const int64_t* sei1, int64_t S,
                        const float* distance, const int64_t* noise_level, const float* distance_noise,
                        const GeosslNcsnWeights* w, int F, float anneal_power, float* loss_e,
                        const GeosslNcsnSaved* saved, float* workspace, hipStream_t stream);
int64_t geossl_loss_reduce_workspace_floats(int64_t S);
int geossl_loss_reduce(const float* loss_e, int64_t S, const int64_t* stats_divisor, float out_scale, float* loss,
                       float* workspace, int accumulate, hipStream_t stream);
typedef struct {
  const float* h;
  const float* distance;
  const int64_t* noise_level;
  const float* distance_noise;
  GeosslNcsnWeights w;
  GeosslNcsnSaved saved;
  float anneal_power;
  float pad_;
  float* loss_e;
  float* workspace;
} GeosslNcsnHeadFwd;
typedef struct {
  const float* h;
  GeosslNcsnWeights w;
  GeosslNcsnSaved saved;
  float out_scale;
  float pad_;
  float* dfeat;
  float* demb;
  float* grow;
  GeosslNcsnGrads grads;
  float* workspace;
  float* dh;
} GeosslNcsnHeadBwd;
int geossl_ddm_loss_fwd2(const GeosslNcsnHeadFwd* heads, const int64_t* batch, const int64_t* sei0, const int64_t* sei1,
                         int64_t S, int F, hipStream_t stream);
int geossl_loss_reduce_partials2(const float* partial0, const float* partial1, const int64_t* stats_divisor, float scale0,
                                 float scale1, float* loss, hipStream_t stream);
int geossl_ddm_loss_bwd_fused2(const GeosslNcsnHeadBwd* heads, const int64_t* sei0, const int64_t* sei1, int64_t S,
                               int64_t N, int F, const int64_t* stats_divisor, const float* gout, const int64_t* inc_ptr,
                               const int32_t* inc_idx, int accumulate, hipStream_t stream);
int geossl_loss_reduce_partials(const float* partial, const int64_t* stats_divisor, float out_scale, float* loss,
                                int accumulate, hipStream_t stream);
int geossl_ddm_loss_bwd_rows(const GeosslNcsnWeights* w, const GeosslNcsnSaved* saved, int64_t S, int F,
                             const int64_t* stats_divisor, float out_scale, const float* gout, float* dz1,
                             float* dfeat, float* demb, float* grow, hipStream_t stream);
int64_t geossl_ddm_loss_bwd_workspace_floats(int64_t S, int F);
int geossl_ddm_loss_bwd_weights(const float* h, const int64_t* sei0, const int64_t* sei1, int64_t S, int F,
                                const GeosslNcsnWeights* w, const GeosslNcsnSaved* saved, const float* dz1,
                                const float* demb, const float* grow, const GeosslNcsnGrads* grads,
                                float* workspace, int accumulate, hipStream_t stream);
int64_t geossl_ddm_loss_bwd_fused_workspace_floats(int64_t S, int F);
int geossl_ddm_loss_bwd_fused(const float* h, const int64_t* sei0, const int64_t* sei1, int64_t S, int64_t N, int F,
                              const GeosslNcsnWeights* w, const GeosslNcsnSaved* saved, const int64_t* stats_divisor,
                              float out_scale, const float* gout, float* dfeat, float* demb, float* grow,
                              const GeosslNcsnGrads* grads, float* workspace, int accumulate, hipStream_t stream);
int geossl_incidence_gather(const float* dfeat, const int64_t* inc_ptr, const int32_t* inc_idx, int64_t N, int F,
                            float* dh, int accumulate, hipStream_t stream);

int geossl_painn_edge_geom(const float* pos, const int64_t* idx_i, const int64_t* idx_j, int64_t E, float cutoff,
                           const float* offsets, const float* widths, int R, float* dir, float* fcut, float* phi,
                           hipStream_t stream);
int geossl_silu_fwd(const float* u, int64_t n, float* y, hipStream_t stream);
int geossl_silu_bwd(const float* u, const float* dy, int64_t n, float* du, hipStream_t stream);
int geossl_painn_interaction_fwd(const float* q, const float* mu, const float* xc, const int64_t* idx_j,
                                 const int64_t* inc_ptr, const int32_t* inc_idx, const float* phi, const float* fcut,
                                 const float* dir, const float* Wf, const float* bf, int64_t N, int F, int R,
                                 float* q_out, float* mu_out, hipStream_t stream);
int64_t geossl_painn_interaction_bwd_workspace_floats(int64_t N, int F, int R);
int geossl_painn_interaction_bwd(const float* dq_out, const float* dmu_out, const float* mu, const float* xc,
                                 const int64_t* idx_i, const int64_t* inc_ptr, const int32_t* inc_idx, const float* phi,
                                 const float* fcut, const float* dir, const float* Wf, const float* bf, int64_t N, int F,
                                 int R, float* dxc, float* dmu_in, float* dWf, float* dbf, float* workspace,
                                 int accumulate, hipStream_t stream);
int geossl_painn_interaction_fwd_mma(const float* q, const float* mu, const float* xc, const int64_t* idx_j,
                                     const int32_t* row_edge, const int32_t* grp_atom, const int32_t* mol_grp,
                                     const float* phi, const float* fcut, const float* dir, const float* Wf,
                                     const float* bf, const int32_t* mol_ptr, int64_t B, int max_n, int64_t N, int F, int R,
                                     float* q_out, float* mu_out, hipStream_t stream);
int geossl_painn_interaction_fwd_mol(const float* q, const float* mu, const float* xc, const int64_t* idx_j,
                                     const int64_t* inc_ptr, const int32_t* inc_idx, const float* phi, const float* fcut,
                                     const float* dir, const float* Wf, const float* bf, const int32_t* mol_ptr,
                                     int64_t B, int max_n, int64_t N, int F, int R, float* q_out, float* mu_out,
                                     hipStream_t stream);
int64_t geossl_painn_interaction_bwd_mol_workspace_floats(int64_t N, int64_t B, int F, int R);
int geossl_painn_interaction_bwd_mol(const float* dq_out, const float* dmu_out, const float* mu, const float* xc,
                                     const int64_t* idx_i, const int64_t* inc_ptr, const int32_t* inc_idx,
                                     const float* phi, const float* fcut, const float* dir, const float* Wf,
                                     const float* bf, const int32_t* mol_ptr, int64_t B, int max_n, int64_t N, int F,
                                     int R, float* dxc, float* dmu_in, float* dWf, float* dbf, float* workspace,
                                     int accumulate, hipStream_t stream);
int geossl_painn_mix_pre_fwd(const float* q, const float* mm, int64_t N, int F, float eps, float* ctx, float* dot,
                             hipStream_t stream);
int geossl_painn_mix_post_fwd(const float* q, const float* mu, const float* mm, const float* xx, const float* dot,
                              int64_t N, int F, float* q_out, float* mu_out, hipStream_t stream);
int geossl_painn_mix_post_bwd(const float* dq_new, const float* dmu_new, const float* mm, const float* xx,
                              const float* dot, int64_t N, int F, float* dxx, float* dmm, hipStream_t stream);
int geossl_painn_mix_pre_bwd(const float* dq_new, const float* dctx, const float* ctx, const float* mm, int64_t N, int F,
                             float* dq_in, float* dmm, hipStream_t stream);
int geossl_add(const float* a, const float* b, int64_t n, float* out, hipStream_t stream);

int geossl_painn_edge_grads(const float* dq_out, const float* dmu_out, const float* mu, const float* xc,
                            const int64_t* idx_i, const int64_t* idx_j, const float* phi, const float* fcut,
                            const float* dir, const float* Wf, const float* bf, int64_t E, int F, int R, float* dphi,
                            float* dfcut, float* ddir, int accumulate, hipStream_t stream);
int geossl_painn_edge_geom_bwd(const float* pos, const int64_t* idx_i, const int64_t* idx_j, int64_t E, float cutoff,
                               const float* offsets, const float* widths, int R, const float* dphi, const float* dfcut,
                               const float* ddir, float* dr, hipStream_t stream);
int geossl_painn_position_grad(const float* dr, const int64_t* inc_i_ptr, const int32_t* inc_i_idx,
                               const int64_t* inc_j_ptr, const int32_t* inc_j_idx, int64_t N, float* dpos,
                               hipStream_t stream);

int geossl_adam_step(float* param, const float* grad, float* exp_avg, float* exp_avg_sq, int64_t n, double lr,
                     double beta1, double beta2, double eps, double weight_decay, int64_t step_count, float grad_scale,
                     hipStream_t stream);

#define GEOSSL_COPY_MAX 8
typedef struct GeosslCopyBatch {
  void* dst[GEOSSL_COPY_MAX];
  const void* src[GEOSSL_COPY_MAX];
  int64_t bytes[GEOSSL_COPY_MAX];
} GeosslCopyBatch;
int geossl_copy_n(const GeosslCopyBatch* batch, int n, hipStream_t stream);
int geossl_ddm_views_dyn(const float* pos, const float* noise, const int64_t* sei0, const int64_t* sei1, int64_t N,
                         int64_t S, float* pos2, float* d01, float* d02, const int64_t* z, int64_t z_stride, int64_t* z2,
                         const int32_t* dyn_N, const int32_t* dyn_S, hipStream_t stream);
int geossl_embedding_fwd_dyn(const int64_t* z, int64_t z_stride, const float* table, int num_classes, int64_t N, int F,
                             float* out, int32_t* status, const int32_t* dyn_N, hipStream_t stream);
int geossl_embedding_bwd_dyn(const int64_t* z, int64_t z_stride, const float* dh, int num_classes, int64_t N, int F,
                             float* dtable, float* workspace, int accumulate, const int32_t* dyn_N, hipStream_t stream);
int geossl_cfconv_filter_fwd_dyn(const float* pair_d, const float* pair_c, int64_t P, const GeosslFilterWeights* w, int L,
                                 int F, int G, const float* offset, float coeff, float* T, float* Wf,
                                 const int32_t* dyn_P, hipStream_t stream);
int geossl_cfconv_filter_bwd_dyn(const float* pair_d, const float* pair_c, const uint8_t* pair_flag,
                                 const int32_t* pair_i, const int32_t* pair_j, int64_t P, int64_t N,
                                 const GeosslFilterWeights* w, const GeosslFilterGradIn* g, int L, int F, int G,
                                 const float* offset, float coeff, const float* T, const GeosslFilterGradOut* out,
                                 float* workspace, int accumulate, const int32_t* dyn_P, const int32_t* dyn_N,
                                 hipStream_t stream);
int geossl_cfconv_aggregate_work_dyn(const float* x, const float* Wf, const uint8_t* pair_flag, const int32_t* mol_ptr,
                                     const int32_t* pair_ptr, const int32_t* work, int64_t nwork, int max_n, int F,
                                     int swap, float* out, const int32_t* dyn_nwork, hipStream_t stream);
int geossl_linear_chain_dyn(const float* X, int ldx, const GeosslChain* chain, int64_t R, int F, const int32_t* dyn_R,
                            hipStream_t stream);
int geossl_linear_wgrad_dyn(const GeosslTnBatch* batch, int nprob, int64_t R, int M, int N, int lda, int ldb, int ldw,
                            float* workspace, int accumulate, const int32_t* dyn_R, hipStream_t stream);
int geossl_ddm_loss_fwd2_dyn(const GeosslNcsnHeadFwd* heads, const int64_t* batch, const int64_t* sei0,
                             const int64_t* sei1, int64_t S, int F, const int32_t* dyn_S, const int32_t* dyn_view,
                             hipStream_t stream);
int geossl_ddm_loss_bwd_fused2_dyn(const GeosslNcsnHeadBwd* heads, const int64_t* sei0, const int64_t* sei1, int64_t S,
                                   int64_t N, int F, const int64_t* stats_divisor, const float* gout,
                                   const int64_t* inc_ptr, const int32_t* inc_idx, int accumulate, const int32_t* dyn_S,
                                   const int32_t* dyn_view, hipStream_t stream);

int64_t geossl_painn_group_capacity(int64_t E2, int64_t N2);
int geossl_painn_edge_layout(const int64_t* src_i, const int64_t* src_j, int64_t E, const int32_t* mol_ptr, int64_t N,
                             int64_t B, int64_t N2cap, int64_t* idx_i2, int64_t* idx_j2, int64_t* iptr_i,
                             int32_t* ilist_i, int64_t* iptr_j, int32_t* ilist_j, int32_t* row_edge, int32_t* grp_atom,
                             int32_t* mol_grp, int32_t* mol_grp_end, int32_t* status, hipStream_t stream);
int geossl_painn_edge_layout_dyn(const int64_t* src_i, const int64_t* src_j, int64_t E_cap, const int32_t* dyn_E,
                                 const int32_t* mol_ptr, int64_t N, int64_t B, int64_t N2cap, int64_t* idx_i2,
                                 int64_t* idx_j2, int64_t* iptr_i, int32_t* ilist_i, int64_t* iptr_j, int32_t* ilist_j,
                                 int32_t* row_edge, int32_t* grp_atom, int32_t* mol_grp, int32_t* mol_grp_end,
                                 int32_t* status, hipStream_t stream);
int geossl_painn_edge_geom_dyn(const float* pos, const int64_t* idx_i, const int64_t* idx_j, int64_t E, float cutoff,
                               const float* offsets, const float* widths, int R, float* dir, float* fcut, float* phi,
                               const int32_t* dyn_E, hipStream_t stream);
int geossl_painn_interaction_fwd_mma_dyn(const float* q, const float* mu, const float* xc, const int64_t* idx_j,
                                         const int32_t* row_edge, const int32_t* grp_atom, const int32_t* mol_grp,
                                         const float* phi, const float* fcut, const float* dir, const float* Wf,
                                         const float* bf, const int32_t* mol_ptr, int64_t B, int max_n, int64_t N, int F,
                                         int R, float* q_out, float* mu_out, const int32_t* mol_grp_end,
                                         hipStream_t stream);
int geossl_painn_stage_cap(int kind, int F, int R);
int geossl_painn_interaction_fwd_atoms(const float* q, const float* mu, const float* xc, const int64_t* idx_j,
                                       const int64_t* inc_ptr, const int32_t* inc_idx, const float* phi,
                                       const float* fcut, const float* dir, const float* Wf, const float* bf,
                                       const int32_t* atom_list, int64_t nlist, const int32_t* dyn_nlist, int F, int R,
                                       float* q_out, float* mu_out, hipStream_t stream);
int geossl_painn_interaction_bwd_atoms(const float* dq_out, const float* dmu_out, const float* mu, const float* xc,
                                       const int64_t* idx_i, const int64_t* inc_ptr, const int32_t* inc_idx,
                                       const float* phi, const float* fcut, const float* dir, const float* Wf,
                                       const float* bf, const int32_t* atom_list, int64_t nlist,
                                       const int32_t* dyn_nlist, int F, int R, float* dxc, float* dmu_in, float* dWf,
                                       float* dbf, float* workspace, int accumulate, hipStream_t stream);
int geossl_painn_interaction_bwd_mol_skip(const float* dq_out, const float* dmu_out, const float* mu, const float* xc,
                                          const int64_t* idx_i, const int64_t* inc_ptr, const int32_t* inc_idx,
                                          const float* phi, const float* fcut, const float* dir, const float* Wf,
                                          const float* bf, const int32_t* mol_ptr, int64_t B, int max_n, int64_t N, int F,
                                          int R, float* dxc, float* dmu_in, float* dWf, float* dbf, float* workspace,
                                          int accumulate, hipStream_t stream);
int geossl_painn_mix_pre_fwd_dyn(const float* q, const float* mm, int64_t N, int F, float eps, float* ctx, float* dot,
                                 const int32_t* dyn_N, hipStream_t stream);
int geossl_painn_mix_post_fwd_dyn(const float* q, const float* mu, const float* mm, const float* xx, const float* dot,
                                  int64_t N, int F, float* q_out, float* mu_out, const int32_t* dyn_N,
                                  hipStream_t stream);
int geossl_painn_mix_post_bwd_dyn(const float* dq_new, const float* dmu_new, const float* mm, const float* xx,
                                  const float* dot, int64_t N, int F, float* dxx, float* dmm, const int32_t* dyn_N,
                                  hipStream_t stream);
int geossl_painn_mix_pre_bwd_dyn(const float* dq_new, const float* dctx, const float* ctx, const float* mm, int64_t N,
                                 int F, float* dq_in, float* dmm, const int32_t* dyn_N, hipStream_t stream);

int geossl_tape_unary(int kind, const float* x, int64_t n, float alpha, float beta, float* y, hipStream_t stream);
int geossl_tape_binary(int op, const float* a, int amode, const float* b, int bmode, int64_t R, int D, float scale,
                       float* y, hipStream_t stream);
int64_t geossl_tape_colsum_workspace_floats(int64_t R, int D);
int geossl_tape_reduce(int kind, const float* x, int64_t R, int D, float* y, float* workspace, hipStream_t stream);
int geossl_tape_gather_rows(const float* src, const void* idx, int idx64, int64_t E, int D, float* out,
                            hipStream_t stream);
int geossl_tape_scatter_rows(const float* src, const void* ptr, int ptr64, const int32_t* perm, int64_t N, int D,
                             float* out, hipStream_t stream);
int geossl_tape_copy2d(const float* src, int64_t ld_src, float* dst, int64_t ld_dst, int64_t R, int C,
                       hipStream_t stream);
int geossl_tape_fill(float* dst, int64_t n, float value, hipStream_t stream);

typedef struct GeosslGather {
  const int64_t* x_src;
  const float* pos_src;
  const int32_t* src_off;
  const int32_t* mol_ptr;
  int64_t* x_dst;
  float* pos_dst;
  int64_t* batch_dst;
  const int32_t* se_ptr;
  int64_t* sei0;
  int64_t* sei1;
  const int32_t* pair_ptr2;
  int32_t* pair_i;
  int32_t* pair_j;
  const int64_t* inc_ptr;
  int32_t* inc_idx;
  const int64_t* e0_src;
  const int64_t* e1_src;
  const int32_t* e_src_off;
  const int32_t* e_ptr;
  int64_t* e0_dst;
  int64_t* e1_dst;
  float* zero;
  int64_t zero_count;
  int32_t x_cols;
  int32_t option;
} GeosslGather;
int geossl_gather_molecules(const GeosslGather* g, int64_t B, hipStream_t stream);

typedef struct GeosslMask {
  const int32_t* bond_ptr;
  const int32_t* bond_dst;
  const int32_t* src_n;
  const int64_t* mol_id;
  const int32_t* keep_in;
  int32_t* keep_out;
  const int32_t* e_src_cnt;
  int32_t* e_count;
  uint64_t seed;
  int32_t max_n;
  int32_t pad_;
} GeosslMask;
int geossl_gather_masked_molecules(const GeosslGather* g, const GeosslMask* mask, int64_t B, hipStream_t stream);

int geossl_masked_edge_offsets(const int32_t* e_count, int64_t B, int64_t E_cap, int views, int32_t* e_ptr,
                               int32_t* dyn_E2, int32_t* status, hipStream_t stream);

int geossl_infonce_fwd(const float* X, const float* Y, int64_t B, int F, float inv_t, float* stats, int32_t* amax,
                       float* loss, int32_t* counts, hipStream_t stream);
int geossl_infonce_bwd(const float* X, const float* Y, const float* stats, const int32_t* amax, int64_t B, int F,
                       float inv_t, const float* gout, float* dX, float* dY, hipStream_t stream);
int geossl_ebm_nce_fwd(const float* X, const float* Y, int64_t B, int F, int num_neg, float* pred, double* terms,
                       int32_t* hits, double* loss, int32_t* counts, hipStream_t stream);
int geossl_ebm_nce_bwd(const float* X, const float* Y, const float* pred, int64_t B, int F, int num_neg,
                       const double* gout, float* dX, float* dY, hipStream_t stream);

int geossl_distance_head_width_ok(int F);
int64_t geossl_distance_head_fwd_workspace_floats(int64_t S);
int64_t geossl_distance_head_bwd_workspace_floats(int64_t N, int F);
int geossl_distance_head_fwd(const float* h, int64_t N, int F, const float* W, const float* bias, const float* pos,
                             const int64_t* sei0, const int64_t* sei1, int64_t S, float* proj, float* pred, float* sgn,
                             float* workspace, float* loss, hipStream_t stream);
int geossl_distance_head_fwd_dyn(const float* h, int64_t N, int F, const float* W, const float* bias, const float* pos,
                                 const int64_t* sei0, const int64_t* sei1, int64_t S, float* proj, float* pred,
                                 float* sgn, float* workspace, float* loss, const int32_t* dyn_N, const int32_t* dyn_S,
                                 hipStream_t stream);
int geossl_distance_head_bwd(const float* h, int64_t N, int F, const float* W, const int64_t* sei0, int64_t S,
                             const float* sgn, const int64_t* inc_ptr, const int32_t* inc_idx, const float* gout,
                             float* dh, float* dW, float* db, float* workspace, int accumulate, hipStream_t stream);
int geossl_distance_head_bwd_dyn(const float* h, int64_t N, int F, const float* W, const int64_t* sei0, int64_t S,
                                 const float* sgn, const int64_t* inc_ptr, const int32_t* inc_idx, const float* gout,
                                 float* dh, float* dW, float* db, float* workspace, int accumulate,
                                 const int32_t* dyn_N, const int32_t* dyn_S, hipStream_t stream);

int64_t geossl_charge_mask_count(int64_t N, double ratio);
int geossl_charge_mask(int64_t* x, int x_cols, int64_t N, double ratio, int C, int64_t* seed, const int64_t* given,
                       int64_t* idx, int64_t* labels, int32_t* k, hipStream_t stream);
int geossl_charge_mask_dyn(int64_t* x, int x_cols, int64_t N, double ratio, int C, int64_t* seed, const int64_t* given,
                           int64_t* idx, int64_t* labels, int32_t* k, const int32_t* dyn_N, hipStream_t stream);
int geossl_charge_head_width_ok(int F, int C);
int64_t geossl_charge_head_fwd_workspace_floats(int64_t K);
int64_t geossl_charge_head_bwd_workspace_floats(int64_t K, int F, int C);
int geossl_charge_head_fwd(const float* h, int64_t N, int F, const float* W, const float* bias, int C,
                           const int64_t* idx, const int64_t* labels, int64_t K, const int32_t* k_dev, float* prob,
                           float* workspace, float* loss, int32_t* status, hipStream_t stream);
int geossl_charge_head_fwd_dyn(const float* h, int64_t N, int F, const float* W, const float* bias, int C,
                               const int64_t* idx, const int64_t* labels, int64_t K, const int32_t* k_dev, float* prob,
                               float* workspace, float* loss, int32_t* status, const int32_t* dyn_N,
                               hipStream_t stream);
int geossl_charge_head_bwd(const float* h, int64_t N, int F, const float* W, int C, const int64_t* idx,
                           const int64_t* labels, int64_t K, const int32_t* k_dev, const float* prob, const float* gout,
                           float* dh, float* dW, float* db, float* workspace, int accumulate, hipStream_t stream);
int geossl_charge_head_bwd_dyn(const float* h, int64_t N, int F, const float* W, int C, const int64_t* idx,
                               const int64_t* labels, int64_t K, const int32_t* k_dev, const float* prob,
                               const float* gout, float* dh, float* dW, float* db, float* workspace, int accumulate,
                               const int32_t* dyn_N, hipStream_t stream);

int geossl_infograph_width_ok(int F);
int64_t geossl_infograph_fwd_workspace_floats(int64_t B);
int geossl_infograph_fwd(const float* x, int64_t N, int F, const float* W, const int32_t* mol_ptr, int64_t B,
                         int readout, const float* m_in, float* s, float* h, float* scores, float* workspace,
                         float* loss, int32_t* counts, hipStream_t stream);
int geossl_infograph_fwd_dyn(const float* x, int64_t N, int F, const float* W, const int32_t* mol_ptr, int64_t B,
                             int readout, const float* m_in, float* s, float* h, float* scores, float* workspace,
                             float* loss, int32_t* counts, const int32_t* dyn_N, hipStream_t stream);
int geossl_infograph_bwd(const float* x, int64_t N, int F, const float* W, const int32_t* mol_ptr, int64_t B,
                         int readout, const float* s, const float* h, const float* scores, const float* gout,
                         float* dx, float* dm, float* dh, hipStream_t stream);
int geossl_infograph_bwd_dyn(const float* x, int64_t N, int F, const float* W, const int32_t* mol_ptr, int64_t B,
                             int readout, const float* s, const float* h, const float* scores, const float* gout,
                             float* dx, float* dm, float* dh, const int32_t* dyn_N, hipStream_t stream);

int geossl_property_width_ok(int F);
int64_t geossl_property_workspace_floats(int64_t B);
int geossl_property_fwd(const float* h, int64_t N, int F, const int32_t* mol_ptr, int64_t B, int readout, int head,
                        const float* W1, const float* b1, const float* W2, const float* b2, const float* y,
                        int64_t y_stride, const float* stats, int loss_kind, float* m, float* z, float* pred,
                        float* workspace, float* loss, hipStream_t stream);
int geossl_property_fwd_dyn(const float* h, int64_t N, int F, const int32_t* mol_ptr, int64_t B, int readout, int head,
                            const float* W1, const float* b1, const float* W2, const float* b2, const float* y,
                            int64_t y_stride, const float* stats, int loss_kind, float* m, float* z, float* pred,
                            float* workspace, float* loss, const int32_t* dyn_N, hipStream_t stream);
int geossl_property_predict(const float* h, int64_t N, int F, const int32_t* mol_ptr, int64_t B, int readout, int head,
                            const float* W1, const float* b1, const float* W2, const float* b2, const float* stats,
                            float* pred, hipStream_t stream);
int geossl_property_predict_dyn(const float* h, int64_t N, int F, const int32_t* mol_ptr, int64_t B, int readout,
                                int head, const float* W1, const float* b1, const float* W2, const float* b2,
                                const float* stats, float* pred, const int32_t* dyn_N, hipStream_t stream);
int geossl_property_bwd(int64_t N, int F, const int32_t* mol_ptr, int64_t B, int readout, int head, const float* W1,
                        const float* W2, const float* m, const float* z, const float* pred, const float* y,
                        int64_t y_stride, const float* stats, int loss_kind, const float* gout, float* dh, float* dz,
                        float* dw, float* db, float* workspace, int accumulate, hipStream_t stream);
int geossl_property_bwd_dyn(int64_t N, int F, const int32_t* mol_ptr, int64_t B, int readout, int head, const float* W1,
                            const float* W2, const float* m, const float* z, const float* pred, const float* y,
                            int64_t y_stride, const float* stats, int loss_kind, const float* gout, float* dh, float* dz,
                            float* dw, float* db, float* workspace, int accumulate, const int32_t* dyn_N,
                            hipStream_t stream);
int geossl_property_targets(const float* y, int64_t M, int T, int task_id, const int64_t* mol_off,
                            const int32_t* src_off, int64_t B, float* out, hipStream_t stream);

int geossl_pair_head_width_ok(int F);
int64_t geossl_pair_head_workspace_floats(int64_t B);
int geossl_pair_head_fwd(const float* h, int64_t N, int F, const int32_t* mol_ptr, int64_t B, int readout, const float* w,
                         const float* b, const float* y, float* m, float* z, float* workspace, float* loss,
                         hipStream_t stream);
int geossl_pair_head_predict(const float* h, int64_t N, int F, const int32_t* mol_ptr, int64_t B, int readout,
                             const float* w, const float* b, float* z, hipStream_t stream);
int geossl_pair_head_bwd(int64_t N, int F, const int32_t* mol_ptr, int64_t B, int readout, const float* w, const float* m,
                         const float* z, const float* y, const float* gout, float* dh, float* dw, float* db,
                         float* workspace, int accumulate, hipStream_t stream);

int geossl_torsion_head_width_ok(int F);
int64_t geossl_torsion_head_fwd_workspace_floats(int64_t T);
int64_t geossl_torsion_head_bwd_workspace_floats(int64_t N, int F);
int geossl_torsion_head_fwd(const float* h, int64_t N, int F, const float* W, const float* bias, const int64_t* tri0,
                            const int64_t* tri1, const int64_t* tri2, const float* angle, int64_t T, float* proj,
                            float* pred, float* res, float* workspace, float* loss, hipStream_t stream);
int geossl_torsion_head_fwd_dyn(const float* h, int64_t N, int F, const float* W, const float* bias, const int64_t* tri0,
                                const int64_t* tri1, const int64_t* tri2, const float* angle, int64_t T, float* proj,
                                float* pred, float* res, float* workspace, float* loss, const int32_t* dyn_N,
                                const int32_t* dyn_T, hipStream_t stream);
int geossl_torsion_head_bwd(const float* h, int64_t N, int F, const float* W, const int64_t* tri0, const int64_t* tri1,
                            const int64_t* tri2, int64_t T, const float* res, const int32_t* mol_ptr, int64_t B,
                            const float* gout, float* dh, float* dW, float* db, float* workspace, int accumulate,
                            hipStream_t stream);
int geossl_torsion_head_bwd_dyn(const float* h, int64_t N, int F, const float* W, const int64_t* tri0,
                                const int64_t* tri1, const int64_t* tri2, int64_t T, const float* res,
                                const int32_t* mol_ptr, int64_t B, const float* gout, float* dh, float* dW, float* db,
                                float* workspace, int accumulate, const int32_t* dyn_N, const int32_t* dyn_T,
                                hipStream_t stream);
int geossl_triple_angles(const float* pos, int64_t N, const int64_t* tri0, const int64_t* tri1, const int64_t* tri2,
                         int64_t T, float* angle, hipStream_t stream);
int geossl_gather_triples(const int32_t* tri_src, int64_t stride, const float* angle_src, const int32_t* t_src_off,
                          const int32_t* t_ptr, const int32_t* mol_ptr, int64_t B, int64_t* tri0, int64_t* tri1,
                          int64_t* tri2, float* angle_dst, hipStream_t stream);

int geossl_sparse_pairs_build(const float* pos, const int32_t* mol_ptr, int64_t B, int64_t N, int max_n, float r2,
                              int cap, float cutoff, int64_t capacity, int32_t* mol_cnt, int32_t* up_cnt,
                              int32_t* lo_cnt, int32_t* pair_i, int32_t* pair_j, float* pair_d, float* pair_c,
                              uint8_t* pair_flag, int32_t* inc_ptr, int32_t* inc_pair, uint32_t* inc_src,
                              int32_t* n_pairs, hipStream_t stream);

int geossl_pair_geometry_live(const float* pos, const int32_t* mol_ptr, const int32_t* pair_ptr, int64_t B, int max_n,
                              float r2, int cap, float cutoff, float* pair_d, float* pair_c, uint8_t* pair_flag,
                              int32_t* mol_live, hipStream_t stream);
int geossl_live_pairs_build(const float* pair_d, const float* pair_c, const uint8_t* pair_flag, const int32_t* pair_i,
                            const int32_t* pair_j, const int32_t* mol_ptr, const int32_t* pair_ptr,
                            const int32_t* mol_live, int64_t B, int64_t P, float cutoff, const int32_t* dyn_P,
                            float* live_d, float* live_c, uint8_t* live_flag, int32_t* live_i, int32_t* live_j,
                            int32_t* row_slot, int32_t* n_live, hipStream_t stream);
int geossl_cfconv_filter_fwd_rows(const float* pair_d, const float* pair_c, int64_t P, const GeosslFilterWeights* w, int L,
                                  int F, int G, const float* offset, float coeff, float* T, float* Wf,
                                  const int32_t* dyn_P, const int32_t* row_slot, hipStream_t stream);
int geossl_gather_live_rows(const float* src, const int32_t* row_slot, const int32_t* n_live, int64_t P, int L, int F,
                            float* dst, hipStream_t stream);

int geossl_cfconv_aggregate_sparse(const float* x, const float* Wf, const int32_t* inc_ptr, const int32_t* inc_pair,
                                   const uint32_t* inc_src, int64_t N, int F, int swap, float* out,
                                   hipStream_t stream);
int geossl_pair_position_grad_sparse(const float* pos, const float* pair_d, const float* dd, const int32_t* inc_ptr,
                                     const int32_t* inc_pair, const uint32_t* inc_src, int64_t N, int64_t P, int L,
                                     float* dpos, hipStream_t stream);

#ifdef __cplusplus
}
#endif
#endif
```

Baseline: 410,200.

## Project NCSN first layer per atom before gathering edge pairs

The NCSN score head's first linear layer on the summed atom features of each edge (h_u + h_v) is now rewritten as W·h_u + W·h_v. A new kernel computes W·h once per atom with bf16-split MFMA, and the loss forward gathers the projected rows, skipping the per-edge first-layer GEMM. This moves most of the first-layer FLOPs from edges to atoms, which are fewer, at the cost of an extra per-atom buffer, one more launch and a slightly different floating-point summation order. It is enabled by default unless certain env switches are set or the sizes would overflow 32-bit offsets.

Result: no change. 408,900 (median of 3 runs) (-0.3%).

```diff
diff --git a/geossl_amd/NCSN.py b/geossl_amd/NCSN.py
--- a/geossl_amd/NCSN.py
+++ b/geossl_amd/NCSN.py
@@ -64,6 +64,11 @@
         for ev, _keep in _SIDE["pending"]:
             torch.cuda.current_stream().wait_event(ev)
         _SIDE["pending"].clear()
+
+
+def _per_atom_forward(S, N, Fd):
+    return (_env("GEOSSL_NCSN_PER_EDGE") is None and _env("GEOSSL_NCSN_SPLIT_BWD") is None
+            and _env("GEOSSL_ARITH_24BIT") is None and max(S, N) * Fd * 4 < 2 ** 32)
 
 
 class _NcsnLoss(torch.autograd.Function):
@@ -93,7 +98,13 @@
         nws = max(int(lib.geossl_ddm_loss_fwd_workspace_floats(Fd)), 256)
         ws = (torch.empty if S > 0 else torch.zeros)(nws, dtype=torch.float32, device=dev)
         st = stream()
-        call("geossl_ddm_loss_fwd", ptr(h), ptr(sel.batch), ptr(sel.sei0), ptr(sel.sei1), S,
+        if _per_atom_forward(S, h.size(0), Fd) and S > 0:
+            a = torch.empty_like(h)
+            call("geossl_ncsn_atom_proj", ptr(h), ptr(ps[4]), h.size(0), Fd, ptr(a), st)
+            entry, x = "geossl_ddm_loss_fwd_atom", a
+        else:
+            entry, x = "geossl_ddm_loss_fwd", h
+        call(entry, ptr(x), ptr(sel.batch), ptr(sel.sei0), ptr(sel.sei1), S,
              ptr(distance.contiguous()), ptr(noise_level.contiguous()), ptr(distance_noise.contiguous()), C.byref(w),
              Fd, float(anneal_power), ptr(loss_e), C.byref(sv) if sv is not None else None, ptr(ws), st)
         loss = torch.empty((), dtype=torch.float32, device=dev)
@@ -207,8 +218,17 @@
             saved.append(sv)
             ws.append(w_)
         st = stream()
-        call("geossl_ddm_loss_fwd2_dyn", C.byref(heads), ptr(sel.batch), ptr(sel.sei0), ptr(sel.sei1), S, Fd,
-             None if dyn is None else dyn.n_super, None if dyn is None else dyn.n_atoms, st)
+        if _per_atom_forward(S, N, Fd):
+            Na = sel.N if dyn is not None else N
+            a = torch.empty(2, Na, Fd, dtype=torch.float32, device=dev)
+            call("geossl_ncsn_atom_proj2_dyn", ptr(hs[0]), ptr(hs[1]), ptr(pss[0][4]), ptr(pss[1][4]), Na, Fd, ptr(a[0]),
+                 ptr(a[1]), None if dyn is None else dyn.n_atoms, st)
+            heads[0].h, heads[1].h = ptr(a[0]), ptr(a[1])
+            call("geossl_ddm_loss_fwd_atom2_dyn", C.byref(heads), ptr(sel.batch), ptr(sel.sei0), ptr(sel.sei1), S, Fd,
+                 None if dyn is None else dyn.n_super, st)
+        else:
+            call("geossl_ddm_loss_fwd2_dyn", C.byref(heads), ptr(sel.batch), ptr(sel.sei0), ptr(sel.sei1), S, Fd,
+                 None if dyn is None else dyn.n_super, None if dyn is None else dyn.n_atoms, st)
         loss = torch.empty((), dtype=torch.float32, device=dev)
         call("geossl_loss_reduce_partials2", ptr(ws[0]), ptr(ws[1]), ptr(sel.stats), float(out_scale), float(out_scale),
              ptr(loss), st)
diff --git a/geossl_amd/_lib.py b/geossl_amd/_lib.py
--- a/geossl_amd/_lib.py
+++ b/geossl_amd/_lib.py
@@ -205,6 +205,12 @@
     "geossl_linear_chain_dyn": (i32, [vp, i32, P(Chain), i64, i32, vp, vp]),
     "geossl_linear_wgrad_dyn": (i32, [P(TnBatch), i32, i64, i32, i32, i32, i32, i32, vp, i32, vp, vp]),
     "geossl_ddm_loss_fwd2_dyn": (i32, [vp, vp, vp, vp, i64, i32, vp, vp, vp]),
+    "geossl_ncsn_atom_proj": (i32, [vp, vp, i64, i32, vp, vp]),
+    "geossl_ncsn_atom_proj2": (i32, [vp, vp, vp, vp, i64, i32, vp, vp, vp]),
+    "geossl_ncsn_atom_proj2_dyn": (i32, [vp, vp, vp, vp, i64, i32, vp, vp, vp, vp]),
+    "geossl_ddm_loss_fwd_atom": (i32, [vp, vp, vp, vp, i64, vp, vp, vp, P(NcsnWeights), i32, f32, vp, P(NcsnSaved), vp, vp]),
+    "geossl_ddm_loss_fwd_atom2": (i32, [vp, vp, vp, vp, i64, i32, vp]),
+    "geossl_ddm_loss_fwd_atom2_dyn": (i32, [vp, vp, vp, vp, i64, i32, vp, vp]),
     "geossl_ddm_loss_bwd_fused2_dyn": (i32, [vp, vp, vp, i64, i64, i32, vp, vp, vp, vp, i32, vp, vp, vp]),
     "geossl_painn_group_capacity": (i64, [i64, i64]),
     "geossl_painn_edge_layout": (i32, [vp, vp, i64, vp, i64, i64, i64] + [vp] * 12),
diff --git a/geossl_amd/build.py b/geossl_amd/build.py
--- a/geossl_amd/build.py
+++ b/geossl_amd/build.py
@@ -16,7 +16,7 @@
 SOURCE_FLAGS = {"painn_mma.hip": ["-fno-slp-vectorize"], "distance_head.hip": ["-fno-slp-vectorize"],
                 "charge_head.hip": ["-fno-slp-vectorize"], "infograph_head.hip": ["-fno-slp-vectorize"],
                 "property_head.hip": ["-fno-slp-vectorize"], "torsion_head.hip": ["-fno-slp-vectorize"],
-                "pair_head.hip": ["-fno-slp-vectorize"]}
+                "pair_head.hip": ["-fno-slp-vectorize"], "ncsn_atom.hip": ["-fno-slp-vectorize"]}
 
 
 def _headers():
diff --git a/geossl_amd/csrc/ncsn_atom.hip b/geossl_amd/csrc/ncsn_atom.hip
--- /dev/null
+++ b/geossl_amd/csrc/ncsn_atom.hip
@@ -0,0 +1,221 @@
+#include "common.h"
+#include "geossl_hip.h"
+#include "split.h"
+#include "ncsn_fwd.h"
+
+using namespace geossl;
+
+namespace {
+
+struct NcsnProjHead {
+  const float* h;
+  const float* o1_w;
+  float* a;
+};
+struct NcsnProjPair { NcsnProjHead a[2]; };
+template <int NMB>
+__global__ __launch_bounds__(512) void k_ncsn_atom_proj(NcsnProjPair pr, int N, const int32_t* __restrict__ dyn_view) {
+  constexpr int F = 32 * NMB, KS = F / 16;
+  extern __shared__ __attribute__((aligned(16))) uint8_t smem_raw[];
+  u32x4* W1f = reinterpret_cast<u32x4*>(smem_raw);
+  const NcsnProjHead& a = pr.a[blockIdx.y];
+  const int tid = threadIdx.x, lane = tid & 63, wave = tid >> 6, j = lane & 31, kh = lane >> 5;
+  const float* h = a.h;
+  if (dyn_view != nullptr && blockIdx.y == 1) h += (size_t)(*dyn_view) * F;
+  N = dyn_count(N, dyn_view);
+  const int nrb = (N + 31) / 32;
+  if ((int)blockIdx.x * 8 >= nrb) return;
+  for (int i = tid; i < NMB * KS * 64; i += 512) {
+    const int ln = i & 63, ks = (i >> 6) % KS, mb = i / (64 * KS);
+    const float* row = a.o1_w + (size_t)(32 * mb + (ln & 31)) * (F + 1) + 16 * ks + 8 * (ln >> 5);
+    float v[8];
+#pragma unroll
+    for (int e = 0; e < 8; ++e) v[e] = row[e];
+    const Frag3 f = split8(v);
+    u32x4* dst = W1f + ((size_t)(mb * KS + ks) * 3) * 64 + ln;
+    dst[0] = f.h;
+    dst[64] = f.m;
+    dst[128] = f.l;
+  }
+  __syncthreads();
+  for (int rb = blockIdx.x * 8 + wave; rb < nrb; rb += gridDim.x * 8) {
+    const int row = 32 * rb + j;
+    const bool valid = row < N;
+    const float* hr = h + (size_t)min(row, N - 1) * F + 8 * kh;
+    f32x4 g[KS][2];
+#pragma unroll
+    for (int ks = 0; ks < KS; ++ks) {
+      g[ks][0] = *reinterpret_cast<const f32x4*>(hr + 16 * ks);
+      g[ks][1] = *reinterpret_cast<const f32x4*>(hr + 16 * ks + 4);
+    }
+    f32x16 acc[NMB];
+#pragma unroll
+    for (int mb = 0; mb < NMB; ++mb)
+#pragma unroll
+      for (int r = 0; r < 16; ++r) acc[mb][r] = 0.0f;
+#pragma unroll
+    for (int ks = 0; ks < KS; ++ks) {
+      const float v[8] = {g[ks][0].x, g[ks][0].y, g[ks][0].z, g[ks][0].w, g[ks][1].x, g[ks][1].y, g[ks][1].z, g[ks][1].w};
+      const Frag3 bf = split8(v);
+      Frag3 af[NMB];
+#pragma unroll
+      for (int mb = 0; mb < NMB; ++mb) {
+        const u32x4* src = W1f + ((size_t)(mb * KS + ks) * 3) * 64 + lane;
+        af[mb].h = src[0];
+        af[mb].m = src[64];
+        af[mb].l = src[128];
+      }
+#pragma unroll
+      for (int mb = 0; mb < NMB; ++mb) acc[mb] = mfma_bf16(af[mb].l, bf.h, acc[mb]);
+#pragma unroll
+      for (int mb = 0; mb < NMB; ++mb) acc[mb] = mfma_bf16(af[mb].h, bf.l, acc[mb]);
+#pragma unroll
+      for (int mb = 0; mb < NMB; ++mb) acc[mb] = mfma_bf16(af[mb].m, bf.m, acc[mb]);
+#pragma unroll
+      for (int mb = 0; mb < NMB; ++mb) acc[mb] = mfma_bf16(af[mb].m, bf.h, acc[mb]);
+#pragma unroll
+      for (int mb = 0; mb < NMB; ++mb) acc[mb] = mfma_bf16(af[mb].h, bf.m, acc[mb]);
+#pragma unroll
+      for (int mb = 0; mb < NMB; ++mb) acc[mb] = mfma_bf16(af[mb].h, bf.h, acc[mb]);
+      __builtin_amdgcn_sched_barrier(0);
+    }
+    if (valid) {
+      float* arow = a.a + (size_t)row * F + 4 * kh;
+#pragma unroll
+      for (int mb = 0; mb < NMB; ++mb)
+#pragma unroll
+        for (int q = 0; q < 4; ++q)
+          *reinterpret_cast<f32x4*>(arow + 32 * mb + 8 * q) =
+              f32x4{acc[mb][4 * q], acc[mb][4 * q + 1], acc[mb][4 * q + 2], acc[mb][4 * q + 3]};
+    }
+  }
+}
+
+template <int NMB>
+__global__ __launch_bounds__(512) void k_ncsn_fwd_atom(const float* __restrict__ a, const int64_t* __restrict__ batch,
+                                                       const int64_t* __restrict__ sei0,
+                                                       const int64_t* __restrict__ sei1, int S,
+                                                       const float* __restrict__ distance,
+                                                       const int64_t* __restrict__ noise_level,
+                                                       const float* __restrict__ dist_noise, GeosslNcsnWeights w,
+                                                       float anneal_power, float* __restrict__ loss_e,
+                                                       GeosslNcsnSaved sv, float* __restrict__ loss_part) {
+  ncsn_fwd_body<NMB, true>(a, batch, sei0, sei1, S, distance, noise_level, dist_noise, w, anneal_power, loss_e, sv,
+                           loss_part);
+}
+template <int NMB>
+__global__ __launch_bounds__(512) void k_ncsn_fwd_atom2(NcsnFwdPair pr, const int64_t* __restrict__ batch,
+                                                        const int64_t* __restrict__ sei0,
+                                                        const int64_t* __restrict__ sei1, int S,
+                                                        const int32_t* __restrict__ dyn_S) {
+  const NcsnFwdHead& a = pr.a[blockIdx.y];
+  ncsn_fwd_body<NMB, true>(a.h, batch, sei0, sei1, dyn_count(S, dyn_S), a.distance, a.noise_level, a.dist_noise, a.w,
+                           a.anneal_power, a.loss_e, a.sv, a.loss_part);
+}
+
+}
+
+namespace {
+inline size_t fwd_atom_lds(int F) {
+  const int H = F / 2, HMB = (H + 31) / 32, KS = F / 16;
+  return (size_t)HMB * KS * 3 * 1024 + (size_t)(5 * F + 2 * 32 * HMB + 8) * sizeof(float);
+}
+int launch_atom_proj(const NcsnProjPair& pr, int nheads, int64_t N, int F, const int32_t* dyn_view, hipStream_t stream) {
+  if (N <= 0) return 0;
+  if (F != 32 && F != 64 && F != 128) return (int)hipErrorInvalidValue;
+  for (int k = 0; k < nheads; ++k)
+    if (pr.a[k].h == nullptr || pr.a[k].o1_w == nullptr || pr.a[k].a == nullptr) return (int)hipErrorInvalidValue;
+  const int NMB = F / 32, KS = F / 16;
+  const size_t lds = (size_t)NMB * KS * 3 * 1024;
+  const int nrb = (int)((N + 31) / 32);
+  int nx = (nrb + 7) / 8;
+  if (nx > 128) nx = 128;
+  dim3 grid(nx, nheads);
+#define LAUNCH(NMBV)                                                                                          \
+  do {                                                                                                        \
+    allow_big_lds(&k_ncsn_atom_proj<NMBV>);                                                                   \
+    hipLaunchKernelGGL((k_ncsn_atom_proj<NMBV>), grid, dim3(512), lds, stream, pr, (int)N, dyn_view);         \
+  } while (0)
+  if (F == 128) LAUNCH(4); else if (F == 64) LAUNCH(2); else LAUNCH(1);
+#undef LAUNCH
+  GEOSSL_CHECK_LAUNCH();
+  return 0;
+}
+}
+
+extern "C" int geossl_ncsn_atom_proj(const float* h, const float* o1_w, int64_t N, int F, float* a, hipStream_t stream) {
+  NcsnProjPair pr;
+  pr.a[0] = NcsnProjHead{h, o1_w, a};
+  pr.a[1] = pr.a[0];
+  return launch_atom_proj(pr, 1, N, F, nullptr, stream);
+}
+
+extern "C" int geossl_ncsn_atom_proj2(const float* h0, const float* h1, const float* o1_w0, const float* o1_w1,
+                                      int64_t N, int F, float* a0, float* a1, hipStream_t stream) {
+  return geossl_ncsn_atom_proj2_dyn(h0, h1, o1_w0, o1_w1, N, F, a0, a1, nullptr, stream);
+}
+
+extern "C" int geossl_ncsn_atom_proj2_dyn(const float* h0, const float* h1, const float* o1_w0, const float* o1_w1,
+                                          int64_t N, int F, float* a0, float* a1, const int32_t* dyn_view,
+                                          hipStream_t stream) {
+  NcsnProjPair pr;
+  pr.a[0] = NcsnProjHead{h0, o1_w0, a0};
+  pr.a[1] = NcsnProjHead{h1, o1_w1, a1};
+  return launch_atom_proj(pr, 2, N, F, dyn_view, stream);
+}
+
+extern "C" int geossl_ddm_loss_fwd_atom(const float* a, const int64_t* batch, const int64_t* sei0, const int64_t* sei1,
+                                        int64_t S, const float* distance, const int64_t* noise_level,
+                                        const float* distance_noise, const GeosslNcsnWeights* w, int F,
+                                        float anneal_power, float* loss_e, const GeosslNcsnSaved* saved,
+                                        float* workspace, hipStream_t stream) {
+  if (S <= 0) return 0;
+  if (F != 32 && F != 64 && F != 128) return (int)hipErrorInvalidValue;
+  GeosslNcsnSaved sv = {nullptr, nullptr, nullptr, nullptr, nullptr};
+  if (saved != nullptr) sv = *saved;
+  const size_t lds = fwd_atom_lds(F);
+  dim3 grid(row_blocks_grid(S));
+#define LAUNCH(NMBV)                                                                                                 \
+  do {                                                                                                               \
+    allow_big_lds(&k_ncsn_fwd_atom<NMBV>);                                                                           \
+    hipLaunchKernelGGL((k_ncsn_fwd_atom<NMBV>), grid, dim3(512), lds, stream, a, batch, sei0, sei1, (int)S, distance, \
+                       noise_level, distance_noise, *w, anneal_power, loss_e, sv, workspace);                        \
+  } while (0)
+  if (F == 128) LAUNCH(4); else if (F == 64) LAUNCH(2); else LAUNCH(1);
+#undef LAUNCH
+  GEOSSL_CHECK_LAUNCH();
+  return 0;
+}
+
+extern "C" int geossl_ddm_loss_fwd_atom2(const GeosslNcsnHeadFwd* heads, const int64_t* batch, const int64_t* sei0,
+                                         const int64_t* sei1, int64_t S, int F, hipStream_t stream) {
+  return geossl_ddm_loss_fwd_atom2_dyn(heads, batch, sei0, sei1, S, F, nullptr, stream);
+}
+
+extern "C" int geossl_ddm_loss_fwd_atom2_dyn(const GeosslNcsnHeadFwd* heads, const int64_t* batch, const int64_t* sei0,
+                                             const int64_t* sei1, int64_t S, int F, const int32_t* dyn_S,
+                                             hipStream_t stream) {
+  if (S <= 0) return 0;
+  if (heads == nullptr || (F != 32 && F != 64 && F != 128)) return (int)hipErrorInvalidValue;
+  NcsnFwdPair pr;
+  NcsnFwdHead* a = pr.a;
+  for (int k = 0; k < 2; ++k) {
+    const GeosslNcsnHeadFwd& hd = heads[k];
+    if (hd.h == nullptr || hd.loss_e == nullptr) return (int)hipErrorInvalidValue;
+    a[k].h = hd.h; a[k].distance = hd.distance; a[k].noise_level = hd.noise_level; a[k].dist_noise = hd.distance_noise;
+    a[k].w = hd.w; a[k].sv = hd.saved; a[k].anneal_power = hd.anneal_power; a[k].loss_e = hd.loss_e;
+    a[k].loss_part = hd.workspace;
+  }
+  const size_t lds = fwd_atom_lds(F);
+  dim3 grid((row_blocks_grid(S) + 1) / 2, 2);
+#define LAUNCH(NMBV)                                                                                              \
+  do {                                                                                                            \
+    allow_big_lds(&k_ncsn_fwd_atom2<NMBV>);                                                                       \
+    hipLaunchKernelGGL((k_ncsn_fwd_atom2<NMBV>), grid, dim3(512), lds, stream, pr, batch, sei0, sei1, (int)S,      \
+                       dyn_S);                                                                                    \
+  } while (0)
+  if (F == 128) LAUNCH(4); else if (F == 64) LAUNCH(2); else LAUNCH(1);
+#undef LAUNCH
+  GEOSSL_CHECK_LAUNCH();
+  return 0;
+}
diff --git a/geossl_amd/csrc/ncsn_fwd.h b/geossl_amd/csrc/ncsn_fwd.h
--- /dev/null
+++ b/geossl_amd/csrc/ncsn_fwd.h
@@ -0,0 +1,327 @@
+#pragma once
+#include "common.h"
+#include "geossl_hip.h"
+#include "split.h"
+
+namespace {
+using namespace geossl;
+
+struct RowIn {
+  int64_t u, v;
+  float sigma, d, eps;
+};
+
+template <int NMB, bool PER_ATOM = false>
+__device__ __forceinline__ void ncsn_fwd_body(const float* __restrict__ h, const int64_t* __restrict__ batch,
+                                              const int64_t* __restrict__ sei0, const int64_t* __restrict__ sei1,
+                                              int S, const float* __restrict__ distance,
+                                              const int64_t* __restrict__ noise_level,
+                                              const float* __restrict__ dist_noise, const GeosslNcsnWeights& w,
+                                              float anneal_power, float* __restrict__ loss_e,
+                                              const GeosslNcsnSaved& sv, float* __restrict__ loss_part) {
+  constexpr int F = 32 * NMB, H = F / 2, HMB = (H + 31) / 32, HP = 32 * HMB, KS = F / 16;
+  extern __shared__ __attribute__((aligned(16))) uint8_t smem_raw[];
+  u32x4* W1f = reinterpret_cast<u32x4*>(smem_raw);
+  u32x4* W2f = W1f + (PER_ATOM ? 0 : NMB * KS * 3 * 64);
+  float* b1s = reinterpret_cast<float*>(W2f + HMB * KS * 3 * 64);
+  float* wls = b1s + F;
+  float* b2s = wls + F;
+  float* w3s = b2s + HP;
+  float* iw1 = w3s + HP;
+  float* ib1 = iw1 + F;
+  float* iw2 = ib1 + F;
+  float* lred = iw2 + F;
+  const int tid = threadIdx.x, lane = tid & 63, wave = tid >> 6, j = lane & 31, kh = lane >> 5;
+  const int nrb = (S + 31) / 32;
+  float lsum = 0.0f;
+  auto load_row = [&](int rb) {
+    RowIn r;
+    const int rowc = min(32 * rb + j, S - 1);
+    r.u = sei0[rowc];
+    r.v = sei1[rowc];
+    r.sigma = w.sigmas[noise_level[batch[r.u]]];
+    r.d = distance[rowc];
+    r.eps = dist_noise[rowc];
+    return r;
+  };
+  int rb = blockIdx.x + gridDim.x * wave;
+  RowIn cur;
+  if (rb < nrb) cur = load_row(rb);
+#ifdef NCSN_STAGE_UNROLL
+#pragma unroll
+#endif
+  for (int i = tid; i < (PER_ATOM ? 0 : NMB * KS * 64); i += 512) {
+    const int ln = i & 63, ks = (i >> 6) % KS, mb = i / (64 * KS);
+    const float* row = w.o1_w + (size_t)(32 * mb + (ln & 31)) * (F + 1) + 16 * ks + 8 * (ln >> 5);
+    float v[8];
+#pragma unroll
+    for (int e = 0; e < 8; ++e) v[e] = row[e];
+    const Frag3 f = split8(v);
+    u32x4* dst = W1f + ((size_t)(mb * KS + ks) * 3) * 64 + ln;
+    dst[0] = f.h;
+    dst[64] = f.m;
+    dst[128] = f.l;
+  }
+#ifdef NCSN_STAGE_UNROLL
+#pragma unroll
+#endif
+  for (int i = tid; i < HMB * KS * 64; i += 512) {
+    const int ln = i & 63, ks = (i >> 6) % KS, mb = i / (64 * KS);
+    const int m = 32 * mb + (ln & 31);
+    const float* row = w.o2_w + (size_t)min(m, H - 1) * F + 16 * ks + 4 * (ln >> 5);
+    const f32x4 lo = *reinterpret_cast<const f32x4*>(row), hi = *reinterpret_cast<const f32x4*>(row + 8);
+    float v[8] = {lo.x, lo.y, lo.z, lo.w, hi.x, hi.y, hi.z, hi.w};
+    if (m >= H) {
+#pragma unroll
+      for (int e = 0; e < 8; ++e) v[e] = 0.0f;
+    }
+    const Frag3 f = split8(v);
+    u32x4* dst = W2f + ((size_t)(mb * KS + ks) * 3) * 64 + ln;
+    dst[0] = f.h;
+    dst[64] = f.m;
+    dst[128] = f.l;
+  }
+  for (int i = tid; i < F; i += 512) {
+    b1s[i] = w.o1_b[i];
+    wls[i] = w.o1_w[(size_t)i * (F + 1) + F];
+    iw1[i] = w.in_w1[i];
+    ib1[i] = w.in_b1[i];
+    iw2[i] = w.in_w2[i];
+  }
+  for (int i = tid; i < HP; i += 512) {
+    b2s[i] = i < H ? w.o2_b[i] : 0.0f;
+    w3s[i] = i < H ? w.o3_w[i] : 0.0f;
+  }
+  __syncthreads();
+  const float ib2 = w.in_b2[0], b3 = w.o3_b[0];
+  for (; rb < nrb; rb += gridDim.x * 8) {
+    const int row = 32 * rb + j;
+    const bool valid = row < S;
+    const RowIn in = cur;
+    f32x4 gq[2][4];
+    f32x4 au[PER_ATOM ? NMB : 1][4], av[PER_ATOM ? NMB : 1][4];
+    auto gather = [&](int ks, f32x4 (&g)[4]) {
+      const float* hu = h + (size_t)in.u * F + 16 * ks + 8 * kh;
+      const float* hv = h + (size_t)in.v * F + 16 * ks + 8 * kh;
+      g[0] = *reinterpret_cast<const f32x4*>(hu);
+      g[1] = *reinterpret_cast<const f32x4*>(hu + 4);
+      g[2] = *reinterpret_cast<const f32x4*>(hv);
+      g[3] = *reinterpret_cast<const f32x4*>(hv + 4);
+    };
+    RowIn nxt;
+    int64_t nxt_mol = 0, nxt_lvl = 0;
+    if constexpr (PER_ATOM) {
+      const int rowc_n = min(32 * (rb + (int)gridDim.x * 8) + j, S - 1);
+      nxt.u = sei0[rowc_n];
+      nxt.v = sei1[rowc_n];
+      nxt.d = distance[rowc_n];
+      nxt.eps = dist_noise[rowc_n];
+      const float* pu = h + (size_t)in.u * F + 4 * kh;
+      const float* pv = h + (size_t)in.v * F + 4 * kh;
+#pragma unroll
+      for (int mb = 0; mb < NMB; ++mb)
+#pragma unroll
+        for (int q = 0; q < 4; ++q) {
+          au[mb][q] = *reinterpret_cast<const f32x4*>(pu + 32 * mb + 8 * q);
+          av[mb][q] = *reinterpret_cast<const f32x4*>(pv + 32 * mb + 8 * q);
+        }
+      __builtin_amdgcn_sched_barrier(0);
+    } else {
+      gather(0, gq[0]);
+    }
+    if constexpr (!PER_ATOM) {
+      if (rb + gridDim.x * 8 < nrb) cur = load_row(rb + gridDim.x * 8);
+    }
+    if constexpr (PER_ATOM) {
+      __builtin_amdgcn_sched_barrier(0);
+      nxt_mol = batch[nxt.u];
+      __builtin_amdgcn_sched_barrier(0);
+    }
+    const float pd = add_rn(in.d, mul_rn(in.eps, in.sigma));
+    float e = 0.0f;
+#pragma unroll 4
+    for (int k = kh * (F / 2); k < (kh + 1) * (F / 2); k += 4) {
+      const f32x4 a = *reinterpret_cast<const f32x4*>(iw1 + k), b = *reinterpret_cast<const f32x4*>(ib1 + k);
+      const f32x4 c = *reinterpret_cast<const f32x4*>(iw2 + k);
+      e = fmaf(c.x, fmaxf(fmaf(a.x, pd, b.x), 0.0f), e);
+      e = fmaf(c.y, fmaxf(fmaf(a.y, pd, b.y), 0.0f), e);
+      e = fmaf(c.z, fmaxf(fmaf(a.z, pd, b.z), 0.0f), e);
+      e = fmaf(c.w, fmaxf(fmaf(a.w, pd, b.w), 0.0f), e);
+    }
+    e += __shfl_xor(e, 32, 64);
+    const float emb = e + ib2;
+    if constexpr (PER_ATOM) {
+      __builtin_amdgcn_sched_barrier(0);
+      nxt_lvl = noise_level[nxt_mol];
+      __builtin_amdgcn_sched_barrier(0);
+    }
+    f32x16 acc1[NMB];
+#pragma unroll
+    for (int mb = 0; mb < (PER_ATOM ? 0 : NMB); ++mb)
+#pragma unroll
+      for (int q = 0; q < 4; ++q) {
+        const f32x4 b = *reinterpret_cast<const f32x4*>(b1s + 32 * mb + 8 * q + 4 * kh);
+        const f32x4 wl = *reinterpret_cast<const f32x4*>(wls + 32 * mb + 8 * q + 4 * kh);
+        acc1[mb][4 * q] = fmaf(emb, wl.x, b.x);
+        acc1[mb][4 * q + 1] = fmaf(emb, wl.y, b.y);
+        acc1[mb][4 * q + 2] = fmaf(emb, wl.z, b.z);
+        acc1[mb][4 * q + 3] = fmaf(emb, wl.w, b.w);
+      }
+#pragma unroll
+    for (int ks = 0; ks < (PER_ATOM ? 0 : KS); ++ks) {
+      if (ks + 1 < KS) gather(ks + 1, gq[(ks + 1) & 1]);
+      const f32x4(&g)[4] = gq[ks & 1];
+      const float v[8] = {g[0].x + g[2].x, g[0].y + g[2].y, g[0].z + g[2].z, g[0].w + g[2].w,
+                          g[1].x + g[3].x, g[1].y + g[3].y, g[1].z + g[3].z, g[1].w + g[3].w};
+      const Frag3 bf = split8(v);
+      Frag3 af[NMB];
+#pragma unroll
+      for (int mb = 0; mb < NMB; ++mb) {
+        const u32x4* src = W1f + ((size_t)(mb * KS + ks) * 3) * 64 + lane;
+        af[mb].h = src[0];
+        af[mb].m = src[64];
+        af[mb].l = src[128];
+      }
+#pragma unroll
+      for (int mb = 0; mb < NMB; ++mb) acc1[mb] = mfma_bf16(af[mb].l, bf.h, acc1[mb]);
+#pragma unroll
+      for (int mb = 0; mb < NMB; ++mb) acc1[mb] = mfma_bf16(af[mb].h, bf.l, acc1[mb]);
+#pragma unroll
+      for (int mb = 0; mb < NMB; ++mb) acc1[mb] = mfma_bf16(af[mb].m, bf.m, acc1[mb]);
+#pragma unroll
+      for (int mb = 0; mb < NMB; ++mb) acc1[mb] = mfma_bf16(af[mb].m, bf.h, acc1[mb]);
+#pragma unroll
+      for (int mb = 0; mb < NMB; ++mb) acc1[mb] = mfma_bf16(af[mb].h, bf.m, acc1[mb]);
+#pragma unroll
+      for (int mb = 0; mb < NMB; ++mb) acc1[mb] = mfma_bf16(af[mb].h, bf.h, acc1[mb]);
+      __builtin_amdgcn_sched_barrier(0);
+    }
+    Frag3 tb[KS];
+    {
+      float* arow = sv.a1 != nullptr ? sv.a1 + (size_t)row * F + 4 * kh : nullptr;
+#pragma unroll
+      for (int mb = 0; mb < NMB; ++mb)
+#pragma unroll
+        for (int half = 0; half < 2; ++half) {
+          float v[8];
+#pragma unroll
+          for (int e2 = 0; e2 < 8; ++e2) v[e2] = fmaxf(acc1[mb][8 * half + e2], 0.0f);
+          if constexpr (PER_ATOM) {
+#pragma unroll
+            for (int q2 = 0; q2 < 2; ++q2) {
+              const int q = 2 * half + q2;
+              const f32x4 b = *reinterpret_cast<const f32x4*>(b1s + 32 * mb + 8 * q + 4 * kh);
+              const f32x4 wl = *reinterpret_cast<const f32x4*>(wls + 32 * mb + 8 * q + 4 * kh);
+              const f32x4 x = au[mb][q], y = av[mb][q];
+              v[4 * q2] = fmaxf(add_rn(add_rn(x.x, y.x), fmaf(emb, wl.x, b.x)), 0.0f);
+              v[4 * q2 + 1] = fmaxf(add_rn(add_rn(x.y, y.y), fmaf(emb, wl.y, b.y)), 0.0f);
+              v[4 * q2 + 2] = fmaxf(add_rn(add_rn(x.z, y.z), fmaf(emb, wl.z, b.z)), 0.0f);
+              v[4 * q2 + 3] = fmaxf(add_rn(add_rn(x.w, y.w), fmaf(emb, wl.w, b.w)), 0.0f);
+            }
+          }
+          if (arow != nullptr && valid) {
+            *reinterpret_cast<f32x4*>(arow + 32 * mb + 16 * half) = f32x4{v[0], v[1], v[2], v[3]};
+            *reinterpret_cast<f32x4*>(arow + 32 * mb + 16 * half + 8) = f32x4{v[4], v[5], v[6], v[7]};
+          }
+          tb[2 * mb + half] = split8(v);
+          __builtin_amdgcn_sched_barrier(0);
+        }
+    }
+    float sc = 0.0f;
+#pragma unroll
+    for (int mb = 0; mb < HMB; ++mb) {
+      f32x16 acc2;
+#pragma unroll
+      for (int q = 0; q < 4; ++q) {
+        const f32x4 b = *reinterpret_cast<const f32x4*>(b2s + 32 * mb + 8 * q + 4 * kh);
+        acc2[4 * q] = b.x;
+        acc2[4 * q + 1] = b.y;
+        acc2[4 * q + 2] = b.z;
+        acc2[4 * q + 3] = b.w;
+      }
+      Frag3 af, an;
+      {
+        const u32x4* src = W2f + ((size_t)(mb * KS) * 3) * 64 + lane;
+        af.h = src[0]; af.m = src[64]; af.l = src[128];
+      }
+#pragma unroll
+      for (int ks = 0; ks < KS; ++ks) {
+        if (ks + 1 < KS) {
+          const u32x4* src = W2f + ((size_t)(mb * KS + ks + 1) * 3) * 64 + lane;
+          an.h = src[0]; an.m = src[64]; an.l = src[128];
+        }
+        __builtin_amdgcn_sched_barrier(0);
+        mma6(acc2, af, tb[ks]);
+        __builtin_amdgcn_sched_barrier(0);
+        if (ks + 1 < KS) af = an;
+      }
+      float* a2row = sv.a2 != nullptr ? sv.a2 + (size_t)row * H + 32 * mb + 4 * kh : nullptr;
+#pragma unroll
+      for (int q = 0; q < 4; ++q) {
+        const f32x4 w3 = *reinterpret_cast<const f32x4*>(w3s + 32 * mb + 8 * q + 4 * kh);
+        const f32x4 a = f32x4{fmaxf(acc2[4 * q], 0.0f), fmaxf(acc2[4 * q + 1], 0.0f), fmaxf(acc2[4 * q + 2], 0.0f),
+                              fmaxf(acc2[4 * q + 3], 0.0f)};
+        sc = fmaf(a.x, w3.x, sc);
+        sc = fmaf(a.y, w3.y, sc);
+        sc = fmaf(a.z, w3.z, sc);
+        sc = fmaf(a.w, w3.w, sc);
+        if (a2row != nullptr && valid && 32 * mb + 8 * q + 4 * kh < H) *reinterpret_cast<f32x4*>(a2row + 8 * q) = a;
+      }
+    }
+    if constexpr (PER_ATOM) {
+      nxt.sigma = w.sigmas[nxt_lvl];
+      __builtin_amdgcn_sched_barrier(0);
+    }
+    sc += __shfl_xor(sc, 32, 64);
+    const float out = sc + b3;
+    const float inv_sigma = 1.0f / in.sigma;
+    const float score = out * inv_sigma;
+    const float target = (-1.0f / (in.sigma * in.sigma)) * (pd - in.d);
+    const float diff = score - target;
+    const float pw = powf(in.sigma, anneal_power);
+    if (valid && kh == 0) {
+      const float le = (0.5f * (diff * diff)) * pw;
+      loss_e[row] = le;
+      lsum += le;
+      if (sv.pd != nullptr) {
+        sv.pd[row] = pd;
+        sv.emb[row] = emb;
+        sv.gscale[row] = diff * pw * inv_sigma;
+      }
+    }
+    if constexpr (PER_ATOM) cur = nxt;
+  }
+  if (loss_part != nullptr) {
+    lsum = wave_sum(lsum);
+    if (lane == 0) lred[wave] = lsum;
+    __syncthreads();
+    if (tid == 0) {
+      float t = 0.0f;
+      for (int i = 0; i < 8; ++i) t += lred[i];
+      loss_part[blockIdx.x] = t;
+    }
+    if (blockIdx.x == 0)
+      for (int i = (int)gridDim.x + tid; i < GEOSSL_LOSS_PARTIALS; i += 512) loss_part[i] = 0.0f;
+  }
+}
+
+struct NcsnFwdHead {
+  const float* h;
+  const float* distance;
+  const int64_t* noise_level;
+  const float* dist_noise;
+  GeosslNcsnWeights w;
+  GeosslNcsnSaved sv;
+  float anneal_power;
+  float* loss_e;
+  float* loss_part;
+};
+struct NcsnFwdPair { NcsnFwdHead a[2]; };
+inline int row_blocks_grid(int64_t S) {
+  const int nrb = (int)((S + 31) / 32);
+  int nx = (nrb + 7) / 8;
+  return nx < 256 ? nx : 256;
+}
+
+
+}
diff --git a/geossl_amd/csrc/ncsn_rows.hip b/geossl_amd/csrc/ncsn_rows.hip
--- a/geossl_amd/csrc/ncsn_rows.hip
+++ b/geossl_amd/csrc/ncsn_rows.hip
@@ -1,258 +1,11 @@
 #include "common.h"
 #include "geossl_hip.h"
 #include "split.h"
+#include "ncsn_fwd.h"
 
 using namespace geossl;
 
 namespace {
-
-struct RowIn {
-  int64_t u, v;
-  float sigma, d, eps;
-};
-
-template <int NMB>
-__device__ __forceinline__ void ncsn_fwd_body(const float* __restrict__ h, const int64_t* __restrict__ batch,
-                                              const int64_t* __restrict__ sei0, const int64_t* __restrict__ sei1,
-                                              int S, const float* __restrict__ distance,
-                                              const int64_t* __restrict__ noise_level,
-                                              const float* __restrict__ dist_noise, const GeosslNcsnWeights& w,
-                                              float anneal_power, float* __restrict__ loss_e,
-                                              const GeosslNcsnSaved& sv, float* __restrict__ loss_part) {
-  constexpr int F = 32 * NMB, H = F / 2, HMB = (H + 31) / 32, HP = 32 * HMB, KS = F / 16;
-  extern __shared__ __attribute__((aligned(16))) uint8_t smem_raw[];
-  u32x4* W1f = reinterpret_cast<u32x4*>(smem_raw);
-  u32x4* W2f = W1f + NMB * KS * 3 * 64;
-  float* b1s = reinterpret_cast<float*>(W2f + HMB * KS * 3 * 64);
-  float* wls = b1s + F;
-  float* b2s = wls + F;
-  float* w3s = b2s + HP;
-  float* iw1 = w3s + HP;
-  float* ib1 = iw1 + F;
-  float* iw2 = ib1 + F;
-  float* lred = iw2 + F;
-  const int tid = threadIdx.x, lane = tid & 63, wave = tid >> 6, j = lane & 31, kh = lane >> 5;
-  const int nrb = (S + 31) / 32;
-  float lsum = 0.0f;
-  auto load_row = [&](int rb) {
-    RowIn r;
-    const int rowc = min(32 * rb + j, S - 1);
-    r.u = sei0[rowc];
-    r.v = sei1[rowc];
-    r.sigma = w.sigmas[noise_level[batch[r.u]]];
-    r.d = distance[rowc];
-    r.eps = dist_noise[rowc];
-    return r;
-  };
-  int rb = blockIdx.x + gridDim.x * wave;
-  RowIn cur;
-  if (rb < nrb) cur = load_row(rb);
-#ifdef NCSN_STAGE_UNROLL
-#pragma unroll
-#endif
-  for (int i = tid; i < NMB * KS * 64; i += 512) {
-    const int ln = i & 63, ks = (i >> 6) % KS, mb = i / (64 * KS);
-    const float* row = w.o1_w + (size_t)(32 * mb + (ln & 31)) * (F + 1) + 16 * ks + 8 * (ln >> 5);
-    float v[8];
-#pragma unroll
-    for (int e = 0; e < 8; ++e) v[e] = row[e];
-    const Frag3 f = split8(v);
-    u32x4* dst = W1f + ((size_t)(mb * KS + ks) * 3) * 64 + ln;
-    dst[0] = f.h;
-    dst[64] = f.m;
-    dst[128] = f.l;
-  }
-#ifdef NCSN_STAGE_UNROLL
-#pragma unroll
-#endif
-  for (int i = tid; i < HMB * KS * 64; i += 512) {
-    const int ln = i & 63, ks = (i >> 6) % KS, mb = i / (64 * KS);
-    const int m = 32 * mb + (ln & 31);
-    const float* row = w.o2_w + (size_t)min(m, H - 1) * F + 16 * ks + 4 * (ln >> 5);
-    const f32x4 lo = *reinterpret_cast<const f32x4*>(row), hi = *reinterpret_cast<const f32x4*>(row + 8);
-    float v[8] = {lo.x, lo.y, lo.z, lo.w, hi.x, hi.y, hi.z, hi.w};
-    if (m >= H) {
-#pragma unroll
-      for (int e = 0; e < 8; ++e) v[e] = 0.0f;
-    }
-    const Frag3 f = split8(v);
-    u32x4* dst = W2f + ((size_t)(mb * KS + ks) * 3) * 64 + ln;
-    dst[0] = f.h;
-    dst[64] = f.m;
-    dst[128] = f.l;
-  }
-  for (int i = tid; i < F; i += 512) {
-    b1s[i] = w.o1_b[i];
-    wls[i] = w.o1_w[(size_t)i * (F + 1) + F];
-    iw1[i] = w.in_w1[i];
-    ib1[i] = w.in_b1[i];
-    iw2[i] = w.in_w2[i];
-  }
-  for (int i = tid; i < HP; i += 512) {
-    b2s[i] = i < H ? w.o2_b[i] : 0.0f;
-    w3s[i] = i < H ? w.o3_w[i] : 0.0f;
-  }
-  __syncthreads();
-  const float ib2 = w.in_b2[0], b3 = w.o3_b[0];
-  for (; rb < nrb; rb += gridDim.x * 8) {
-    const int row = 32 * rb + j;
-    const bool valid = row < S;
-    const RowIn in = cur;
-    f32x4 gq[2][4];
-    auto gather = [&](int ks, f32x4 (&g)[4]) {
-      const float* hu = h + (size_t)in.u * F + 16 * ks + 8 * kh;
-      const float* hv = h + (size_t)in.v * F + 16 * ks + 8 * kh;
-      g[0] = *reinterpret_cast<const f32x4*>(hu);
-      g[1] = *reinterpret_cast<const f32x4*>(hu + 4);
-      g[2] = *reinterpret_cast<const f32x4*>(hv);
-      g[3] = *reinterpret_cast<const f32x4*>(hv + 4);
-    };
-    gather(0, gq[0]);
-    if (rb + gridDim.x * 8 < nrb) cur = load_row(rb + gridDim.x * 8);
-    const float pd = add_rn(in.d, mul_rn(in.eps, in.sigma));
-    float e = 0.0f;
-#pragma unroll 4
-    for (int k = kh * (F / 2); k < (kh + 1) * (F / 2); k += 4) {
-      const f32x4 a = *reinterpret_cast<const f32x4*>(iw1 + k), b = *reinterpret_cast<const f32x4*>(ib1 + k);
-      const f32x4 c = *reinterpret_cast<const f32x4*>(iw2 + k);
-      e = fmaf(c.x, fmaxf(fmaf(a.x, pd, b.x), 0.0f), e);
-      e = fmaf(c.y, fmaxf(fmaf(a.y, pd, b.y), 0.0f), e);
-      e = fmaf(c.z, fmaxf(fmaf(a.z, pd, b.z), 0.0f), e);
-      e = fmaf(c.w, fmaxf(fmaf(a.w, pd, b.w), 0.0f), e);
-    }
-    e += __shfl_xor(e, 32, 64);
-    const float emb = e + ib2;
-    f32x16 acc1[NMB];
-#pragma unroll
-    for (int mb = 0; mb < NMB; ++mb)
-#pragma unroll
-      for (int q = 0; q < 4; ++q) {
-        const f32x4 b = *reinterpret_cast<const f32x4*>(b1s + 32 * mb + 8 * q + 4 * kh);
-        const f32x4 wl = *reinterpret_cast<const f32x4*>(wls + 32 * mb + 8 * q + 4 * kh);
-        acc1[mb][4 * q] = fmaf(emb, wl.x, b.x);
-        acc1[mb][4 * q + 1] = fmaf(emb, wl.y, b.y);
-        acc1[mb][4 * q + 2] = fmaf(emb, wl.z, b.z);
-        acc1[mb][4 * q + 3] = fmaf(emb, wl.w, b.w);
-      }
-#pragma unroll
-    for (int ks = 0; ks < KS; ++ks) {
-      if (ks + 1 < KS) gather(ks + 1, gq[(ks + 1) & 1]);
-      const f32x4(&g)[4] = gq[ks & 1];
-      const float v[8] = {g[0].x + g[2].x, g[0].y + g[2].y, g[0].z + g[2].z, g[0].w + g[2].w,
-                          g[1].x + g[3].x, g[1].y + g[3].y, g[1].z + g[3].z, g[1].w + g[3].w};
-      const Frag3 bf = split8(v);
-      Frag3 af[NMB];
-#pragma unroll
-      for (int mb = 0; mb < NMB; ++mb) {
-        const u32x4* src = W1f + ((size_t)(mb * KS + ks) * 3) * 64 + lane;
-        af[mb].h = src[0];
-        af[mb].m = src[64];
-        af[mb].l = src[128];
-      }
-#pragma unroll
-      for (int mb = 0; mb < NMB; ++mb) acc1[mb] = mfma_bf16(af[mb].l, bf.h, acc1[mb]);
-#pragma unroll
-      for (int mb = 0; mb < NMB; ++mb) acc1[mb] = mfma_bf16(af[mb].h, bf.l, acc1[mb]);
-#pragma unroll
-      for (int mb = 0; mb < NMB; ++mb) acc1[mb] = mfma_bf16(af[mb].m, bf.m, acc1[mb]);
-#pragma unroll
-      for (int mb = 0; mb < NMB; ++mb) acc1[mb] = mfma_bf16(af[mb].m, bf.h, acc1[mb]);
-#pragma unroll
-      for (int mb = 0; mb < NMB; ++mb) acc1[mb] = mfma_bf16(af[mb].h, bf.m, acc1[mb]);
-#pragma unroll
-      for (int mb = 0; mb < NMB; ++mb) acc1[mb] = mfma_bf16(af[mb].h, bf.h, acc1[mb]);
-      __builtin_amdgcn_sched_barrier(0);
-    }
-    Frag3 tb[KS];
-    {
-      float* arow = sv.a1 != nullptr ? sv.a1 + (size_t)row * F + 4 * kh : nullptr;
-#pragma unroll
-      for (int mb = 0; mb < NMB; ++mb)
-#pragma unroll
-        for (int half = 0; half < 2; ++half) {
-          float v[8];
-#pragma unroll
-          for (int e2 = 0; e2 < 8; ++e2) v[e2] = fmaxf(acc1[mb][8 * half + e2], 0.0f);
-          if (arow != nullptr && valid) {
-            *reinterpret_cast<f32x4*>(arow + 32 * mb + 16 * half) = f32x4{v[0], v[1], v[2], v[3]};
-            *reinterpret_cast<f32x4*>(arow + 32 * mb + 16 * half + 8) = f32x4{v[4], v[5], v[6], v[7]};
-          }
-          tb[2 * mb + half] = split8(v);
-          __builtin_amdgcn_sched_barrier(0);
-        }
-    }
-    float sc = 0.0f;
-#pragma unroll
-    for (int mb = 0; mb < HMB; ++mb) {
-      f32x16 acc2;
-#pragma unroll
-      for (int q = 0; q < 4; ++q) {
-        const f32x4 b = *reinterpret_cast<const f32x4*>(b2s + 32 * mb + 8 * q + 4 * kh);
-        acc2[4 * q] = b.x;
-        acc2[4 * q + 1] = b.y;
-        acc2[4 * q + 2] = b.z;
-        acc2[4 * q + 3] = b.w;
-      }
-      Frag3 af, an;
-      {
-        const u32x4* src = W2f + ((size_t)(mb * KS) * 3) * 64 + lane;
-        af.h = src[0]; af.m = src[64]; af.l = src[128];
-      }
-#pragma unroll
-      for (int ks = 0; ks < KS; ++ks) {
-        if (ks + 1 < KS) {
-          const u32x4* src = W2f + ((size_t)(mb * KS + ks + 1) * 3) * 64 + lane;
-          an.h = src[0]; an.m = src[64]; an.l = src[128];
-        }
-        __builtin_amdgcn_sched_barrier(0);
-        mma6(acc2, af, tb[ks]);
-        __builtin_amdgcn_sched_barrier(0);
-        if (ks + 1 < KS) af = an;
-      }
-      float* a2row = sv.a2 != nullptr ? sv.a2 + (size_t)row * H + 32 * mb + 4 * kh : nullptr;
-#pragma unroll
-      for (int q = 0; q < 4; ++q) {
-        const f32x4 w3 = *reinterpret_cast<const f32x4*>(w3s + 32 * mb + 8 * q + 4 * kh);
-        const f32x4 a = f32x4{fmaxf(acc2[4 * q], 0.0f), fmaxf(acc2[4 * q + 1], 0.0f), fmaxf(acc2[4 * q + 2], 0.0f),
-                              fmaxf(acc2[4 * q + 3], 0.0f)};
-        sc = fmaf(a.x, w3.x, sc);
-        sc = fmaf(a.y, w3.y, sc);
-        sc = fmaf(a.z, w3.z, sc);
-        sc = fmaf(a.w, w3.w, sc);
-        if (a2row != nullptr && valid && 32 * mb + 8 * q + 4 * kh < H) *reinterpret_cast<f32x4*>(a2row + 8 * q) = a;
-      }
-    }
-    sc += __shfl_xor(sc, 32, 64);
-    const float out = sc + b3;
-    const float inv_sigma = 1.0f / in.sigma;
-    const float score = out * inv_sigma;
-    const float target = (-1.0f / (in.sigma * in.sigma)) * (pd - in.d);
-    const float diff = score - target;
-    const float pw = powf(in.sigma, anneal_power);
-    if (valid && kh == 0) {
-      const float le = (0.5f * (diff * diff)) * pw;
-      loss_e[row] = le;
-      lsum += le;
-      if (sv.pd != nullptr) {
-        sv.pd[row] = pd;
-        sv.emb[row] = emb;
-        sv.gscale[row] = diff * pw * inv_sigma;
-      }
-    }
-  }
-  if (loss_part != nullptr) {
-    lsum = wave_sum(lsum);
-    if (lane == 0) lred[wave] = lsum;
-    __syncthreads();
-    if (tid == 0) {
-      float t = 0.0f;
-      for (int i = 0; i < 8; ++i) t += lred[i];
-      loss_part[blockIdx.x] = t;
-    }
-    if (blockIdx.x == 0)
-      for (int i = (int)gridDim.x + tid; i < GEOSSL_LOSS_PARTIALS; i += 512) loss_part[i] = 0.0f;
-  }
-}
 
 template <int NMB>
 __global__ __launch_bounds__(512) void k_ncsn_fwd(const float* __restrict__ h, const int64_t* __restrict__ batch,
@@ -264,18 +17,6 @@
                                                   GeosslNcsnSaved sv, float* __restrict__ loss_part) {
   ncsn_fwd_body<NMB>(h, batch, sei0, sei1, S, distance, noise_level, dist_noise, w, anneal_power, loss_e, sv, loss_part);
 }
-struct NcsnFwdHead {
-  const float* h;
-  const float* distance;
-  const int64_t* noise_level;
-  const float* dist_noise;
-  GeosslNcsnWeights w;
-  GeosslNcsnSaved sv;
-  float anneal_power;
-  float* loss_e;
-  float* loss_part;
-};
-struct NcsnFwdPair { NcsnFwdHead a[2]; };
 template <int NMB>
 __global__ __launch_bounds__(512) void k_ncsn_fwd2(NcsnFwdPair pr, const int64_t* __restrict__ batch,
                                                    const int64_t* __restrict__ sei0, const int64_t* __restrict__ sei1,
@@ -479,12 +220,6 @@
       }
     }
   }
-}
-
-inline int row_blocks_grid(int64_t S) {
-  const int nrb = (int)((S + 31) / 32);
-  int nx = (nrb + 7) / 8;
-  return nx < 256 ? nx : 256;
 }
 
 }
diff --git a/include/geossl_hip.h b/include/geossl_hip.h
--- a/include/geossl_hip.h
+++ b/include/geossl_hip.h
@@ -275,6 +275,19 @@
                               const GeosslNcsnWeights* w, const GeosslNcsnSaved* saved, const int64_t* stats_divisor,
                               float out_scale, const float* gout, float* dfeat, float* demb, float* grow,
                               const GeosslNcsnGrads* grads, float* workspace, int accumulate, hipStream_t stream);
+int geossl_ncsn_atom_proj(const float* h, const float* o1_w, int64_t N, int F, float* a, hipStream_t stream);
+int geossl_ncsn_atom_proj2(const float* h0, const float* h1, const float* o1_w0, const float* o1_w1, int64_t N, int F,
+                           float* a0, float* a1, hipStream_t stream);
+int geossl_ncsn_atom_proj2_dyn(const float* h0, const float* h1, const float* o1_w0, const float* o1_w1, int64_t N,
+                               int F, float* a0, float* a1, const int32_t* dyn_view, hipStream_t stream);
+int geossl_ddm_loss_fwd_atom(const float* a, const int64_t* batch, const int64_t* sei0, const int64_t* sei1, int64_t S,
+                             const float* distance, const int64_t* noise_level, const float* distance_noise,
+                             const GeosslNcsnWeights* w, int F, float anneal_power, float* loss_e,
+                             const GeosslNcsnSaved* saved, float* workspace, hipStream_t stream);
+int geossl_ddm_loss_fwd_atom2(const GeosslNcsnHeadFwd* heads, const int64_t* batch, const int64_t* sei0,
+                              const int64_t* sei1, int64_t S, int F, hipStream_t stream);
+int geossl_ddm_loss_fwd_atom2_dyn(const GeosslNcsnHeadFwd* heads, const int64_t* batch, const int64_t* sei0,
+                                  const int64_t* sei1, int64_t S, int F, const int32_t* dyn_S, hipStream_t stream);
 int geossl_incidence_gather(const float* dfeat, const int64_t* inc_ptr, const int32_t* inc_idx, int64_t N, int F,
                             float* dh, int accumulate, hipStream_t stream);
 
```
